# ibm-granite/dolomite-engine

Measured on NVIDIA H100. Metric: tokens_per_sec, higher is better.
Workload: dtype bf16

## Files before the change

dolomite_engine_b200/_lib.py:

```python

from __future__ import annotations

import ctypes
import os
from ctypes import c_char_p, c_float, c_int, c_int64, c_uint32, c_void_p

_HERE = os.path.dirname(os.path.abspath(__file__))
LIB_PATH = os.path.join(_HERE, "lib", "libdolomite_b200.so")


class DolomiteB200Error(RuntimeError):
    pass


_P = c_void_p
_I = c_int
_L = c_int64
_F = c_float
_U = c_uint32

SIGNATURES: dict[str, tuple] = {
    "dolomite_b200_last_error": (c_char_p, []),
    "dolomite_b200_abi_version": (_I, []),
    "dolomite_b200_device_info": (_I, [_P, _P, _P]),
    "dolomite_b200_set_option": (_I, [c_char_p, _I]),
    "dolomite_b200_get_option": (_I, [c_char_p, _P]),
    "dolomite_b200_rmsnorm_fwd": (_I, [_P, _P, _P, _P, _L, _I, _F, _P]),
    "dolomite_b200_rmsnorm_bwd_workspace_bytes": (_L, [_I]),
    "dolomite_b200_rmsnorm_bwd": (_I, [_P, _P, _P, _P, _P, _P, _P, _P, _L, _I, _P]),
    "dolomite_b200_rope_qk_inplace": (_I, [_P, _L, _L, _I, _I, _I, _P, _P, _P, _I, _L, _I, _P]),
    "dolomite_b200_layernorm_fwd": (_I, [_P, _P, _P, _P, _P, _P, _L, _I, _F, _P]),
    "dolomite_b200_layernorm_bwd_workspace_bytes": (_L, [_I]),
    "dolomite_b200_layernorm_bwd": (_I, [_P, _P, _P, _P, _P, _P, _P, _P, _P, _P, _L, _I, _P]),
    "dolomite_b200_act_fwd": (_I, [_I, _I, _P, _P, _L, _L, _P]),
    "dolomite_b200_act_bwd": (_I, [_I, _I, _P, _P, _P, _P, _L, _L, _P]),
    "dolomite_b200_act_bwd_segmented": (_I, [_I, _I, _P, _P, _P, _P, _L, _L, _P, _I, _P]),
    "dolomite_b200_gelu_fwd": (_I, [_P, _P, _L, _P]),
    "dolomite_b200_gelu_bwd": (_I, [_P, _P, _P, _P, _L, _L, _P]),
    "dolomite_b200_swiglu_fwd": (_I, [_P, _P, _L, _L, _P]),
    "dolomite_b200_swiglu_bwd": (_I, [_P, _P, _P, _L, _L, _P]),
    "dolomite_b200_swiglu_bwd_bias": (_I, [_P, _P, _P, _P, _L, _L, _P]),
    "dolomite_b200_embedding_fwd": (_I, [_P, _P, _P, _L, _I, _L, _F, _P]),
    "dolomite_b200_embedding_bwd": (_I, [_P, _P, _P, _L, _I, _L, _F, _P]),
    "dolomite_b200_cross_entropy_fwd_bwd": (_I, [_P, _L, _P, _P, _P, _P, _P, _L, _L, _L, _F, _F, _P]),
    "dolomite_b200_cross_entropy_count": (_I, [_P, _L, _L, _P, _P]),
    "dolomite_b200_cross_entropy_rows": (_I, [_P, _L, _P, _P, _P, _P, _L, _L, _L, _F, _F, _P]),
    "dolomite_b200_cross_entropy_mean": (_I, [_P, _L, _P, _P, _P]),
    "dolomite_b200_colsum_accum": (_I, [_P, _L, _P, _L, _L, _F, _P]),
    "dolomite_b200_colsum_accum_segmented": (_I, [_P, _L, _P, _L, _L, _P, _I, _F, _P]),
    "dolomite_b200_scale_bf16_by_device_scalar": (_I, [_P, _L, _P, _P]),
    "dolomite_b200_add_scaled": (_I, [_P, _P, _P, _F, _L, _P]),
    "dolomite_b200_dropout_fwd": (_I, [_P, _P, _P, _L, _F, _F, _U, _U, _P]),
    "dolomite_b200_dropout_bwd": (_I, [_P, _P, _L, _F, _F, _U, _U, _P]),
    "dolomite_b200_sumsq_workspace_bytes": (_L, []),
    "dolomite_b200_sumsq_accum": (_I, [_P, _L, _P, _P, _P]),
    "dolomite_b200_clip_coef": (_I, [_P, _F, _P, _P, _P]),
    "dolomite_b200_adamw_step": (_I, [_P, _P, _P, _P, _P, _L, _F, _F, _F, _F, _F, _L, _P, _P]),
    "dolomite_b200_cast_f32_to_bf16": (_I, [_P, _P, _L, _P]),
    "dolomite_b200_accum_bf16_into_f32": (_I, [_P, _P, _F, _L, _P]),
    "dolomite_b200_gemm_bf16": (
        _I,
        [_P, _L, _I, _P, _L, _I, _P, _L, _I, _P, _L, _F, _F, _P, _L, _L, _L, _I, _P],
    ),
    "dolomite_b200_gemm_bf16_wgrad_multi": (_I, [_I, _P, _P, _P, _P, _P, _P, _P, _P, _L, _P, _P, _P]),
    "dolomite_b200_gemm_bf16_tile_n": (_I, [_I, _P, _P, _P, _P]),
    "dolomite_b200_gemm_fp8": (
        _I,
        [_P, _L, _I, _P, _L, _I, _P, _P, _P, _L, _I, _P, _L, _F, _F, _P, _L, _L, _L, _I, _P],
    ),
    "dolomite_b200_gemm_fp8_wgrad_multi": (
        _I,
        [_I, _P, _P, _P, _P, _P, _P, _P, _P, _P, _P, _L, _P, _P, _I, _I, _I, _P],
    ),
    "dolomite_b200_fp8_cast": (_I, [_P, _L, _L, _L, _I, _P, _P, _P, _P, _P]),
    "dolomite_b200_fp8_scaling_update": (_I, [_P, _I, _L, _P, _P, _F, _P]),
    "dolomite_b200_gemm_bf16_grouped_m": (_I, [_P, _L, _P, _L, _I, _P, _L, _F, _L, _L, _L, _P, _I, _I, _P]),
    "dolomite_b200_gemm_bf16_grouped_k": (_I, [_P, _L, _P, _L, _P, _L, _F, _F, _L, _L, _L, _P, _I, _P]),
    "dolomite_b200_moe_max_rows": (_L, [_L, _I, _I]),
    "dolomite_b200_moe_route": (_I, [_P, _L, _I, _I, _P, _P, _P, _P, _P, _P, _P, _P, _P, _P]),
    "dolomite_b200_gemm_bf16_grouped_m_gather": (_I, [_P, _L, _L, _P, _P, _L, _P, _L, _F, _L, _L, _L, _P, _I, _I, _P]),
    "dolomite_b200_gemm_bf16_grouped_m_bias": (
        _I,
        [_P, _L, _L, _P, _P, _L, _I, _P, _L, _P, _L, _F, _L, _L, _L, _P, _I, _I, _P],
    ),
    "dolomite_b200_moe_gather": (_I, [_P, _P, _P, _P, _L, _I, _I, _I, _P]),
    "dolomite_b200_moe_combine": (_I, [_P, _P, _P, _P, _P, _L, _I, _I, _F, _P]),
    "dolomite_b200_moe_combine_bwd": (_I, [_P, _P, _P, _P, _P, _P, _P, _L, _I, _I, _I, _F, _P]),
    "dolomite_b200_moe_token_sum": (_I, [_P, _P, _P, _L, _I, _I, _P]),
    "dolomite_b200_moe_router_bwd": (_I, [_P, _P, _P, _P, _L, _I, _I, _P]),
    "dolomite_b200_moe_aux_partial_floats": (_L, [_L, _I]),
    "dolomite_b200_moe_aux_stats": (_I, [_P, _P, _L, _L, _I, _I, _P, _P, _P]),
    "dolomite_b200_moe_aux_finalize": (_I, [_P, _I, _L, _F, _P, _P, _P, _P]),
    "dolomite_b200_moe_router_bwd_aux": (_I, [_P, _P, _P, _P, _P, _P, _P, _L, _L, _I, _I, _P]),
    "dolomite_b200_attn_varlen_fwd": (_I, [_P, _L, _P, _P, _P, _I, _L, _I, _I, _I, _I, _F, _P]),
    "dolomite_b200_attn_decode": (_I, [_P, _L, _P, _P, _P, _P, _I, _L, _I, _I, _I, _F, _P]),
    "dolomite_b200_attn_varlen_bwd_workspace_bytes": (_L, [_L, _I, _I, _I]),
    "dolomite_b200_attn_varlen_bwd": (
        _I,
        [_P, _P, _L, _P, _P, _P, _P, _I, _L, _I, _I, _I, _I, _F, _P, _P],
    ),
    "dolomite_b200_attn_varlen_fwd_dropout": (_I, [_P, _L, _P, _P, _P, _I, _L, _I, _I, _I, _I, _F, _F, _U, _U, _P]),
    "dolomite_b200_attn_varlen_bwd_dropout": (
        _I,
        [_P, _P, _L, _P, _P, _P, _P, _I, _L, _I, _I, _I, _I, _F, _F, _U, _U, _P, _P],
    ),
    "dolomite_b200_attn_varlen_fwd_alibi": (_I, [_P, _L, _P, _P, _P, _I, _L, _I, _I, _I, _I, _F, _F, _U, _U, _P, _P]),
    "dolomite_b200_attn_varlen_bwd_alibi": (
        _I,
        [_P, _P, _L, _P, _P, _P, _P, _I, _L, _I, _I, _I, _I, _F, _F, _U, _U, _P, _P, _P],
    ),
    "dolomite_b200_attn_decode_alibi": (_I, [_P, _L, _P, _P, _P, _P, _I, _L, _I, _I, _I, _F, _P, _P]),
}

_lib = None


def lib_available() -> bool:
    return os.path.exists(LIB_PATH)


def load():
    global _lib
    if _lib is not None:
        return _lib
    if not os.path.exists(LIB_PATH):
        raise DolomiteB200Error(
            f"{LIB_PATH} not found. Build it with `python -m dolomite_engine_b200.build` "
            "(or __graft_entry__.build()); there is no CPU / PyTorch fallback for the hot path."
        )
    lib = ctypes.CDLL(LIB_PATH)
    for name, (res, args) in SIGNATURES.items():
        fn = getattr(lib, name)
        fn.restype = res
        fn.argtypes = args
    _lib = lib
    for item in filter(None, os.environ.get("DOLO_OPTIONS", "").split(",")):
        key, _, value = item.partition("=")
        if lib.dolomite_b200_set_option(key.strip().encode(), int(value)) != 0:
            raise DolomiteB200Error(f"DOLO_OPTIONS: {lib.dolomite_b200_last_error().decode()}")
    return lib


def check(rc: int, what: str = "") -> None:
    if rc != 0:
        msg = load().dolomite_b200_last_error()
        raise DolomiteB200Error(f"{what}: rc={rc}: {msg.decode() if msg else '?'}")


KERNELS_PER_CALL = {
    "dolomite_b200_rmsnorm_fwd": 1, "dolomite_b200_rmsnorm_bwd": 2, "dolomite_b200_rope_qk_inplace": 1,
    "dolomite_b200_layernorm_fwd": 1, "dolomite_b200_layernorm_bwd": 3, "dolomite_b200_gelu_fwd": 1,
    "dolomite_b200_gelu_bwd": 1, "dolomite_b200_swiglu_fwd": 1, "dolomite_b200_swiglu_bwd": 1, "dolomite_b200_swiglu_bwd_bias": 1,
    "dolomite_b200_act_fwd": 1, "dolomite_b200_act_bwd": 1,
    "dolomite_b200_embedding_fwd": 1,
    "dolomite_b200_embedding_bwd": 1, "dolomite_b200_cross_entropy_fwd_bwd": 3, "dolomite_b200_colsum_accum": 1,
    "dolomite_b200_scale_bf16_by_device_scalar": 1, "dolomite_b200_add_scaled": 1, "dolomite_b200_sumsq_accum": 2,
    "dolomite_b200_clip_coef": 1, "dolomite_b200_adamw_step": 1, "dolomite_b200_cast_f32_to_bf16": 1,
    "dolomite_b200_accum_bf16_into_f32": 1, "dolomite_b200_gemm_bf16": 1, "dolomite_b200_attn_varlen_fwd": 1,
    "dolomite_b200_attn_varlen_bwd": 3, "dolomite_b200_attn_varlen_fwd_dropout": 1, "dolomite_b200_attn_varlen_bwd_dropout": 3,
    "dolomite_b200_attn_varlen_fwd_alibi": 1, "dolomite_b200_attn_varlen_bwd_alibi": 3, "dolomite_b200_attn_decode_alibi": 1,
    "dolomite_b200_dropout_fwd": 1, "dolomite_b200_dropout_bwd": 1, "dolomite_b200_gemm_bf16_tile_n": 0,
    "dolomite_b200_moe_aux_stats": 2,
}
launch_counts: dict[str, int] = {}


def reset_launch_counts() -> None:
    launch_counts.clear()


def total_kernel_launches() -> int:
    return sum(KERNELS_PER_CALL.get(k, 1) * v for k, v in launch_counts.items())


def call(name: str, *args):
    lib = load()
    launch_counts[name] = launch_counts.get(name, 0) + 1
    rc = getattr(lib, name)(*args)
    if rc != 0:
        msg = lib.dolomite_b200_last_error()
        raise DolomiteB200Error(f"{name} failed (rc={rc}): {msg.decode() if msg else '?'}")
```

dolomite_engine_b200/csrc/gemm.cu:

```cuda
#include <string.h>

#include "common.cuh"
#include "wgmma.cuh"
#include "../../include/dolomite_b200.h"

using namespace dolo;

namespace {

constexpr int BM = 128;
constexpr int BN = 128;
constexpr int BK = 64;
constexpr int A_STAGE_BYTES = BM * BK * 2;
constexpr int GEMM_THREADS = 384;

constexpr int EPI_SLAB_BYTES = 64 * 128;
constexpr int EPI_BYTES = 2  * 2  * EPI_SLAB_BYTES;
constexpr int EPI_BIAS_BYTES = 2  * 256 * 2;

template <int TN>
struct Ring {
    static_assert(TN == 128 || TN == 256, "tile width 128 or 256");
    static constexpr int STAGES = TN == 256 ? 4 : 6;
    static constexpr int B_BYTES = TN * BK * 2;
    static constexpr int STAGE_BYTES = A_STAGE_BYTES + B_BYTES;
    static constexpr int EPI_OFFSET = STAGES * STAGE_BYTES;
    static constexpr int BIAS_OFFSET = EPI_OFFSET + EPI_BYTES;
    static constexpr int BAR_OFFSET = BIAS_OFFSET + EPI_BIAS_BYTES;
    static constexpr int SMEM_BYTES = 1024  + BAR_OFFSET + 256 ;
    static_assert(EPI_OFFSET % 1024 == 0, "epilogue slabs must stay 1024-byte aligned");
    static_assert((2 * STAGES + 4) * 8 <= 256, "barrier area");
    static_assert(SMEM_BYTES <= 232448, "shared memory budget exceeded (227 KB per block on sm_90)");
};

constexpr int PRODUCER_REGS = 40;
constexpr int CONSUMER_REGS = 232;
static_assert(PRODUCER_REGS * 128 + 2 * CONSUMER_REGS * 128 <= 65536, "register file exceeded");

constexpr double TILE256_COST = 1.65;

constexpr int MAXP = 4;

struct GemmMaps {
    CUtensorMap a[MAXP], b[MAXP], d[MAXP], c[MAXP];
};

struct Problem {
    void* D;
    const void* C;
    const __nv_bfloat16* bias;
    int64_t ldd, ldc;
    int M, N;
    int num_m, num_n, num_kb;
    int group_m;
    int tile_start;
    float alpha, beta;
    uint64_t hint_a, hint_b;
};

struct GemmParams {
    Problem pr[MAXP];
    int n_prob;
    int num_tiles;
    int d_is_f32;
    int grouped;
    const int* m_tile_group;
    const int* a_row_index;
    const void* gather_a;
    int64_t gather_lda;
    int gather_k;
    int b_group_rows;
    const int* group_k_offsets;
    int num_groups;
    int64_t bias_group_stride;
    const float* a_scale_inv[MAXP];
    const float* b_scale_inv[MAXP];
};

struct TileInfo {
    int q;
    int m_blk, n_blk, grp, kb0, kb1;
    bool valid;
};

__device__ __forceinline__ void tile_coords(int t, int num_m, int num_n, int gm, int& m_blk, int& n_blk) {
    const int per_group = gm * num_n;
    const int group = t / per_group;
    const int first_m = group * gm;
    const int gsize = min(num_m - first_m, gm);
    const int r = t - group * per_group;
    m_blk = first_m + r % gsize;
    n_blk = r / gsize;
}

template <bool GROUPED>
__device__ __forceinline__ TileInfo tile_info(int t, const GemmParams& p) {
    TileInfo ti;
    ti.q = 0;
#pragma unroll
    for (int i = 1; i < MAXP; ++i)
        if (i < p.n_prob && t >= p.pr[i].tile_start) ti.q = i;
    const Problem& pr = p.pr[ti.q];
    t -= pr.tile_start;
    ti.grp = 0;
    ti.kb0 = 0;
    ti.kb1 = pr.num_kb;
    ti.valid = true;
    if (GROUPED && p.grouped == 3) {
        const int per = pr.num_m * pr.num_n;
        const int split = t / per;
        tile_coords(t - split * per, pr.num_m, pr.num_n, pr.group_m, ti.m_blk, ti.n_blk);
        const int kb_per = (pr.num_kb + p.num_groups - 1) / p.num_groups;
        ti.kb0 = split * kb_per;
        ti.kb1 = min(pr.num_kb, ti.kb0 + kb_per);
        ti.valid = ti.kb1 > ti.kb0;
    } else if (GROUPED && p.grouped == 2) {
        const int per = pr.num_m * pr.num_n;
        ti.grp = t / per;
        tile_coords(t - ti.grp * per, pr.num_m, pr.num_n, pr.group_m, ti.m_blk, ti.n_blk);
        ti.kb0 = p.group_k_offsets[ti.grp] / BK;
        ti.kb1 = p.group_k_offsets[ti.grp + 1] / BK;
        ti.valid = ti.kb1 > ti.kb0;
    } else {
        tile_coords(t, pr.num_m, pr.num_n, pr.group_m, ti.m_blk, ti.n_blk);
        if (GROUPED && p.grouped == 1) {
            ti.grp = p.m_tile_group[ti.m_blk];
            ti.valid = ti.grp >= 0;
        }
    }
    return ti;
}

struct Epilogue {
    uint8_t* slabs;
    uint32_t* bias;
    uint64_t* c_bar;
    int slab = 0;
    uint32_t c_phase = 0;
    int cw;
    bool leader;

    __device__ __forceinline__ void load_c_prefetch(const CUtensorMap* cmap, int chunk_cols, int col0, int row0, int grp) {
        tma_store_wait_read<0>();
#pragma unroll
        for (int i = 0; i < 2; ++i) {
            const int s = slab ^ i;
            mbar_expect_tx(&c_bar[s], EPI_SLAB_BYTES);
            tma_load_3d(slabs + s * EPI_SLAB_BYTES, cmap, &c_bar[s], col0 + i * chunk_cols, row0, grp);
        }
    }

    __device__ __forceinline__ void begin_tile() {
        if (leader) tma_store_wait_read<0>();
        named_bar_sync(1 + cw, 128);
    }

    __device__ __forceinline__ void reuse_slab(bool has_c, const CUtensorMap* cmap, int col, int row0, int grp) {
        if (leader) {
            tma_store_wait_read<1>();
            if (has_c) {
                mbar_expect_tx(&c_bar[slab], EPI_SLAB_BYTES);
                tma_load_3d(slabs + slab * EPI_SLAB_BYTES, cmap, &c_bar[slab], col, row0, grp);
            }
        }
        named_bar_sync(1 + cw, 128);
    }

    template <int TN, bool F32, bool SCALED>
    __device__ __forceinline__ void store(const float (&acc)[TN / 2], const CUtensorMap* dmap, const CUtensorMap* cmap,
                                          int col0, int row0, int grp, float s, float alpha, float beta, bool has_bias,
                                          bool has_c, bool reduce) {
        constexpr int CHUNK = F32 ? 32 : 64;
        constexpr int NB = CHUNK / 8;
        const int lane = threadIdx.x & 31;
        const int wrow = ((threadIdx.x >> 5) & 3) * 16;
        auto scaled = [s](float a) { return SCALED ? s * a : a; };
#pragma unroll
        for (int ch = 0; ch < TN / CHUNK; ++ch) {
            uint8_t* sl = slabs + slab * EPI_SLAB_BYTES;
            if (ch >= 2) reuse_slab(has_c, cmap, col0 + ch * CHUNK, row0, grp);
            if (has_c) {
                mbar_wait(&c_bar[slab], (c_phase >> slab) & 1u, 4);
                c_phase ^= 1u << slab;
            }
            if constexpr (F32) {
#pragma unroll
                for (int jj = 0; jj < NB; ++jj) {
                    const int j = ch * NB + jj;
                    float b0 = 0.f, b1 = 0.f;
                    if (has_bias) {
                        const uint32_t bv = bias[4 * j + (lane & 3)];
                        b0 = bf16_lo(bv);
                        b1 = bf16_hi(bv);
                    }
#pragma unroll
                    for (int h = 0; h < 2; ++h) {
                        const int r = wrow + 8 * h + (lane >> 2);
                        const int byte = jj * 32 + (lane & 3) * 8;
                        float2* d = reinterpret_cast<float2*>(sl + r * 128 + ((((byte >> 4) ^ (r & 7)) << 4) | (byte & 15)));
                        float v0 = (scaled(acc[4 * j + 2 * h]) + b0) * alpha;
                        float v1 = (scaled(acc[4 * j + 2 * h + 1]) + b1) * alpha;
                        if (has_c) {
                            const float2 c2 = *d;
                            v0 += beta * c2.x;
                            v1 += beta * c2.y;
                        }
                        *d = make_float2(v0, v1);
                    }
                }
            } else {
                const int m = lane >> 3;
                const int r = wrow + 8 * (m & 1) + (lane & 7);
#pragma unroll
                for (int jj = 0; jj < NB; jj += 2) {
                    const uint32_t addr = smem_u32(sl + r * 128 + (((jj + (m >> 1)) ^ (lane & 7)) << 4));
                    uint32_t cv[4], out[4];
                    if (has_c) ldmatrix_x4(addr, cv);
#pragma unroll
                    for (int i = 0; i < 4; ++i) {
                        const int j = ch * NB + jj + (i >> 1), h = i & 1;
                        float b0 = 0.f, b1 = 0.f;
                        if (has_bias) {
                            const uint32_t bv = bias[4 * j + (lane & 3)];
                            b0 = bf16_lo(bv);
                            b1 = bf16_hi(bv);
                        }
                        float v0 = (scaled(acc[4 * j + 2 * h]) + b0) * alpha;
                        float v1 = (scaled(acc[4 * j + 2 * h + 1]) + b1) * alpha;
                        if (has_c) {
                            v0 += beta * bf16_lo(cv[i]);
                            v1 += beta * bf16_hi(cv[i]);
                        }
                        out[i] = pack_bf16(v0, v1);
                    }
                    stmatrix_x4(addr, out);
                }
            }
            issue(dmap, col0 + ch * CHUNK, row0, grp, reduce);
        }
    }

    template <int TN>
    __device__ __forceinline__ void store_zero_f32(const CUtensorMap* dmap, int col0, int row0, int grp) {
        begin_tile();
#pragma unroll 1
        for (int ch = 0; ch < TN / 32; ++ch) {
            if (ch >= 2) reuse_slab(false, nullptr, 0, 0, 0);
            uint4* s = reinterpret_cast<uint4*>(slabs + slab * EPI_SLAB_BYTES);
#pragma unroll
            for (int i = 0; i < EPI_SLAB_BYTES / 16 / 128; ++i) s[(threadIdx.x & 127) + 128 * i] = make_uint4(0u, 0u, 0u, 0u);
            issue(dmap, col0 + ch * 32, row0, grp, false);
        }
    }

    __device__ __forceinline__ void issue(const CUtensorMap* dmap, int col, int row0, int grp, bool reduce) {
        const uint8_t* sl = slabs + slab * EPI_SLAB_BYTES;
        fence_proxy_async_smem();
        named_bar_sync(1 + cw, 128);
        if (leader) {
            if (reduce)
                tma_reduce_add_3d(dmap, sl, col, row0, grp);
            else
                tma_store_3d(dmap, sl, col, row0, grp);
            tma_store_commit();
        }
        slab ^= 1;
    }
};

template <bool A_MN_, bool B_MN_>
struct Bf16Ops {
    static constexpr bool A_MN = A_MN_, B_MN = B_MN_;
    static constexpr int KB_ELEMS = BK;
    static constexpr bool SPLIT = false, SCALED = false, GROUPED = true;
    template <int TN>
    static __device__ __forceinline__ void mma(float (&acc)[TN / 2], uint64_t adesc, uint64_t bdesc, uint32_t scale_d) {
        wgmma_ss<TN, A_MN ? 1 : 0, B_MN ? 1 : 0>(acc, adesc, bdesc, scale_d);
    }
};

template <int FA, int FB, bool SPLIT_>
struct Fp8Ops {
    static constexpr bool A_MN = false, B_MN = false;
    static constexpr int KB_ELEMS = 128;
    static constexpr bool SPLIT = SPLIT_, SCALED = true, GROUPED = false;
    template <int TN>
    static __device__ __forceinline__ void mma(float (&acc)[TN / 2], uint64_t adesc, uint64_t bdesc, uint32_t scale_d) {
        static_assert(TN == 128, "fp8 tiles are 128 wide");
        wgmma_fp8_n128<FA, FB>(acc, adesc, bdesc, scale_d);
    }
};

template <class Op, int TN>
__device__ __forceinline__ void gemm_body(const GemmMaps& maps, const GemmParams& p) {
    constexpr bool A_MN = Op::A_MN, B_MN = Op::B_MN;
    constexpr int STAGES = Ring<TN>::STAGES;
    constexpr int B_STAGE_BYTES = Ring<TN>::B_BYTES;
    constexpr int STAGE_BYTES = Ring<TN>::STAGE_BYTES;
    extern __shared__ uint8_t smem_raw[];
    uint8_t* smem = smem_align_1024(smem_raw);
    uint8_t* smem_a = smem;
    uint8_t* smem_b = smem + STAGES * A_STAGE_BYTES;
    uint64_t* bars = reinterpret_cast<uint64_t*>(smem + Ring<TN>::BAR_OFFSET);
    uint64_t* full_bar = bars;
    uint64_t* empty_bar = bars + STAGES;
    uint64_t* c_bar = bars + 2 * STAGES;

    const int wg = threadIdx.x >> 7;
    const int warp = threadIdx.x >> 5;
    const int lane = threadIdx.x & 31;
    const int num_tiles = p.num_tiles;
    const bool gather = Op::GROUPED && TN == 128 && !A_MN && p.a_row_index != nullptr;

    if (threadIdx.x == 0) {
        for (int q = 0; q < p.n_prob; ++q) {
            if (!gather) tma_prefetch_desc(&maps.a[q]);
            tma_prefetch_desc(&maps.b[q]);
        }
        for (int i = 0; i < STAGES; ++i) {
            mbar_init(&full_bar[i], gather ? 33 : 1);
            mbar_init(&empty_bar[i], 8);
        }
        for (int i = 0; i < 4; ++i) mbar_init(&c_bar[i], 1);
        mbar_fence_init();
    }
    __syncthreads();

    if (wg == 0) {
        if constexpr (TN == 256) setmaxnreg_dec<PRODUCER_REGS>();
        if (warp != 0) return;
        if (gather) {
            const __nv_bfloat16* A = static_cast<const __nv_bfloat16*>(p.gather_a);
            int stage = 0;
            uint32_t phase = 0;
            for (int t = blockIdx.x; t < num_tiles; t += gridDim.x) {
                const TileInfo ti = tile_info<Op::GROUPED>(t, p);
                if (!ti.valid) continue;
                const CUtensorMap* tmap_b = &maps.b[ti.q];
                const int b_outer = ti.grp * p.b_group_rows;
                const int4 src = *reinterpret_cast<const int4*>(p.a_row_index + int64_t(ti.m_blk) * BM + lane * 4);
                const int srow[4] = {src.x, src.y, src.z, src.w};
                for (int kb = ti.kb0; kb < ti.kb1; ++kb) {
                    mbar_wait(&empty_bar[stage], phase ^ 1, 1);
                    uint8_t* sa = smem_a + stage * A_STAGE_BYTES;
                    uint8_t* sb = smem_b + stage * B_STAGE_BYTES;
                    if (lane == 0) {
                        mbar_expect_tx(&full_bar[stage], B_STAGE_BYTES);
                        if (!B_MN) {
                            tma_load_2d(sb, tmap_b, &full_bar[stage], kb * BK, b_outer + ti.n_blk * BN);
                        } else {
#pragma unroll
                            for (int i = 0; i < BN / 64; ++i)
                                tma_load_2d(sb + i * (BK * 128), tmap_b, &full_bar[stage], ti.n_blk * BN + i * 64,
                                            b_outer + kb * BK);
                        }
                    }
#pragma unroll
                    for (int i = 0; i < 4; ++i) {
                        const int r = lane * 4 + i;
                        const __nv_bfloat16* g = A + int64_t(srow[i]) * p.gather_lda + int64_t(kb) * BK;
#pragma unroll
                        for (int c = 0; c < 8; ++c) {
                            uint4 v = make_uint4(0u, 0u, 0u, 0u);
                            if (kb * BK + c * 8 < p.gather_k) v = __ldg(reinterpret_cast<const uint4*>(g + c * 8));
                            *reinterpret_cast<uint4*>(sa + r * 128 + ((c ^ (r & 7)) << 4)) = v;
                        }
                    }
                    fence_proxy_async_smem();
                    mbar_arrive(&full_bar[stage]);
                    if (++stage == STAGES) { stage = 0; phase ^= 1; }
                }
            }
        } else if (elect_one()) {
            int stage = 0;
            uint32_t phase = 0;
            for (int t = blockIdx.x; t < num_tiles; t += gridDim.x) {
                const TileInfo ti = tile_info<Op::GROUPED>(t, p);
                if (!ti.valid) continue;
                const CUtensorMap* tmap_a = &maps.a[ti.q];
                const CUtensorMap* tmap_b = &maps.b[ti.q];
                const uint64_t ha = p.pr[ti.q].hint_a, hb = p.pr[ti.q].hint_b;
                const int m_blk = ti.m_blk, n_blk = ti.n_blk;
                const int b_outer = (Op::GROUPED && p.grouped == 1) ? ti.grp * p.b_group_rows : 0;
                for (int kb = ti.kb0; kb < ti.kb1; ++kb) {
                    mbar_wait(&empty_bar[stage], phase ^ 1, 1);
                    uint8_t* sa = smem_a + stage * A_STAGE_BYTES;
                    uint8_t* sb = smem_b + stage * B_STAGE_BYTES;
                    mbar_expect_tx(&full_bar[stage], STAGE_BYTES);
                    if (!A_MN) {
                        tma_load_2d_hint(sa, tmap_a, &full_bar[stage], kb * Op::KB_ELEMS, m_blk * BM, ha);
                    } else {
#pragma unroll
                        for (int i = 0; i < BM / 64; ++i)
                            tma_load_2d_hint(sa + i * (BK * 128), tmap_a, &full_bar[stage], m_blk * BM + i * 64, kb * BK, ha);
                    }
                    if (!B_MN) {
                        tma_load_2d_hint(sb, tmap_b, &full_bar[stage], kb * Op::KB_ELEMS, b_outer + n_blk * TN, hb);
                    } else {
#pragma unroll
                        for (int i = 0; i < TN / 64; ++i)
                            tma_load_2d_hint(sb + i * (BK * 128), tmap_b, &full_bar[stage], n_blk * TN + i * 64,
                                             b_outer + kb * BK, hb);
                    }
                    if (++stage == STAGES) { stage = 0; phase ^= 1; }
                }
            }
        }
        return;
    }

    if constexpr (TN == 256) setmaxnreg_inc<CONSUMER_REGS>();
    const int cw = wg - 1;
    const int wt = threadIdx.x & 127;
    Epilogue epi;
    epi.slabs = smem + Ring<TN>::EPI_OFFSET + cw * 2 * EPI_SLAB_BYTES;
    epi.bias = reinterpret_cast<uint32_t*>(smem + Ring<TN>::BIAS_OFFSET + cw * (EPI_BIAS_BYTES / 2));
    epi.c_bar = c_bar + 2 * cw;
    epi.cw = cw;
    epi.leader = wt == 0;
    const int chunk_cols = p.d_is_f32 ? 32 : 64;
    int stage = 0;
    uint32_t phase = 0;
    float acc[TN / 2];
    float tot[TN / 2];
    for (int t = blockIdx.x; t < num_tiles; t += gridDim.x) {
        const TileInfo ti = tile_info<Op::GROUPED>(t, p);
        const Problem& pr = p.pr[ti.q];
        const int row0 = ti.m_blk * BM + cw * 64;
        const int col0 = ti.n_blk * TN;
        const int dgrp = Op::GROUPED && p.grouped == 2 ? ti.grp : 0;
        if (!ti.valid) {
            if (Op::GROUPED && p.grouped == 2 && p.d_is_f32 && pr.C == nullptr) epi.store_zero_f32<TN>(&maps.d[ti.q], col0, row0, dgrp);
            continue;
        }
        const bool has_bias = pr.bias != nullptr;
        const bool has_c = pr.C != nullptr;
        uint32_t bias_v = 0;
        if (has_bias && wt < TN / 2 && col0 + 2 * wt < pr.N) {
            const __nv_bfloat16* brow = pr.bias + ti.grp * p.bias_group_stride;
            if (col0 + 2 * wt + 1 < pr.N)
                bias_v = __ldg(reinterpret_cast<const uint32_t*>(brow + col0 + 2 * wt));
            else
                bias_v = __bfloat16_as_ushort(brow[col0 + 2 * wt]);
        }
        int prev_stage = -1;
        for (int kb = ti.kb0; kb < ti.kb1; ++kb) {
            mbar_wait(&full_bar[stage], phase, 3);
            wgmma_fence();
            const uint32_t sa = smem_u32(smem_a + stage * A_STAGE_BYTES);
            const uint32_t sb = smem_u32(smem_b + stage * B_STAGE_BYTES);
#pragma unroll
            for (int k = 0; k < 4; ++k) {
                const uint64_t adesc = A_MN ? gmma_desc(sa + cw * (BK * 128) + k * 2048, BK * 128, 1024, 1)
                                            : gmma_desc(sa + cw * (64 * 128) + k * 32, 16, 1024, 1);
                const uint64_t bdesc = B_MN ? gmma_desc(sb + k * 2048, BK * 128, 1024, 1)
                                            : gmma_desc(sb + k * 32, 16, 1024, 1);
                Op::template mma<TN>(acc, adesc, bdesc, ((!Op::SPLIT && kb != ti.kb0) || k != 0) ? 1u : 0u);
            }
            wgmma_commit();
            if (kb == min(ti.kb0 + 2, ti.kb1 - 1) && has_c && epi.leader) epi.load_c_prefetch(&maps.c[ti.q], chunk_cols, col0, row0, dgrp);
            if constexpr (Op::SPLIT) {
                wgmma_wait<0>();
                reg_fence<TN / 2>(acc);
                if (lane == 0) mbar_arrive(&empty_bar[stage]);
                if (kb == ti.kb0) {
#pragma unroll
                    for (int i = 0; i < TN / 2; ++i) tot[i] = acc[i];
                } else {
#pragma unroll
                    for (int i = 0; i < TN / 2; ++i) tot[i] += acc[i];
                }
            } else {
                wgmma_wait<1>();
                if (prev_stage >= 0 && lane == 0) mbar_arrive(&empty_bar[prev_stage]);
                prev_stage = stage;
            }
            if (++stage == STAGES) { stage = 0; phase ^= 1; }
        }
        if constexpr (!Op::SPLIT) {
            wgmma_wait<0>();
            reg_fence<TN / 2>(acc);
            if (prev_stage >= 0 && lane == 0) mbar_arrive(&empty_bar[prev_stage]);
        }
        const float(&res)[TN / 2] = Op::SPLIT ? tot : acc;
        float s = 1.f;
        if constexpr (Op::SCALED) s = __ldg(p.a_scale_inv[ti.q]) * __ldg(p.b_scale_inv[ti.q]);
        if (has_bias && wt < TN / 2) epi.bias[wt] = bias_v;
        epi.begin_tile();

        if (p.d_is_f32)
            epi.store<TN, true, Op::SCALED>(res, &maps.d[ti.q], &maps.c[ti.q], col0, row0, dgrp, s, pr.alpha, pr.beta,
                                            has_bias, has_c, Op::GROUPED && p.grouped == 3);
        else
            epi.store<TN, false, Op::SCALED>(res, &maps.d[ti.q], &maps.c[ti.q], col0, row0, dgrp, s, pr.alpha, pr.beta,
                                             has_bias, has_c, false);
    }
    if (epi.leader) tma_store_wait_all<0>();
}

template <bool A_MN, bool B_MN, int TN>
__global__ void __launch_bounds__(GEMM_THREADS, 1)
    gemm_bf16_kernel(const __grid_constant__ GemmMaps maps, const __grid_constant__ GemmParams p) {
    gemm_body<Bf16Ops<A_MN, B_MN>, TN>(maps, p);
}

template <int FA, int FB, bool SPLIT>
__global__ void __launch_bounds__(GEMM_THREADS, 1)
    gemm_fp8_kernel(const __grid_constant__ GemmMaps maps, const __grid_constant__ GemmParams p) {
    gemm_body<Fp8Ops<FA, FB, SPLIT>, 128>(maps, p);
}

int gemm_workers() {
    const int sms = dolo_num_sms() - dolo_option_gemm_sm_margin();
    return sms < 1 ? 1 : sms;
}

template <int TN, void (*KERNEL)(GemmMaps, GemmParams)>
int launch_gemm(const GemmMaps& maps, const GemmParams& p, cudaStream_t st) {
    constexpr int smem_bytes = Ring<TN>::SMEM_BYTES;
    static bool attr_set = false;
    if (!attr_set) {
        DOLO_CUDA_OK(cudaFuncSetAttribute(KERNEL, cudaFuncAttributeMaxDynamicSharedMemorySize, smem_bytes));
        attr_set = true;
    }
    const int sms = gemm_workers();
    const int grid = p.num_tiles < sms ? p.num_tiles : sms;
    KERNEL<<<grid, GEMM_THREADS, smem_bytes, st>>>(maps, p);
    DOLO_LAUNCH_OK("gemm");
    return DOLO_OK;
}

int choose_tile_n(int n, const int64_t* M, const int64_t* N) {
    const int forced = dolo_option_gemm_tile_n();
    if (forced != 0) return forced;
    const int64_t w = gemm_workers();
    int64_t t128 = 0, t256 = 0;
    for (int q = 0; q < n; ++q) {
        const int64_t mb = (M[q] + BM - 1) / BM;
        t128 += mb * ((N[q] + 127) / 128);
        t256 += mb * ((N[q] + 255) / 256);
    }
    const double c128 = double((t128 + w - 1) / w);
    const double c256 = double((t256 + w - 1) / w) * TILE256_COST;
    return c256 < c128 ? 256 : 128;
}

}

struct GroupArgs {
    int mode = 0;
    const int* a_row_index = nullptr;
    int64_t a_rows = 0;
    const int* m_tile_group = nullptr;
    int64_t b_group_rows = 0;
    const int* group_k_offsets = nullptr;
    int num_groups = 1;
    int64_t d_group_stride = 0;
    int64_t b_total_outer = 0;
    int64_t bias_group_stride = 0;
};

struct GemmProblemArgs {
    const void* A; int64_t lda;
    const void* B; int64_t ldb;
    void* D; int64_t ldd;
    const void* C; int64_t ldc;
    const void* bias;
    float alpha, beta;
    int64_t M, N, K;
    const float* a_scale_inv = nullptr;
    const float* b_scale_inv = nullptr;
};

static int setup_problem(GemmMaps& maps, GemmParams& p, int q, const GemmProblemArgs& g, int ab, int a_mn_major,
                         int b_mn_major, int d_is_f32, const GroupArgs& ga, int tile_n) {
    const int64_t M = g.M, N = g.N, K = g.K;
    if (ab == 1) {
        DOLO_REQUIRE(M > 0 && N > 0 && K > 0, "gemm_fp8: empty problem (M=%lld N=%lld K=%lld)", (long long)M,
                     (long long)N, (long long)K);
        DOLO_REQUIRE(K % 16 == 0 && N % 16 == 0, "gemm_fp8: K=%lld and N=%lld must be multiples of 16", (long long)K,
                     (long long)N);
        DOLO_REQUIRE(g.lda % 16 == 0 && g.ldb % 16 == 0 && g.lda >= K && g.ldb >= K,
                     "gemm_fp8: lda / ldb must be >= K and multiples of 16 (16-byte aligned fp8 rows)");
        DOLO_REQUIRE(g.a_scale_inv != nullptr && g.b_scale_inv != nullptr, "gemm_fp8: missing scale_inv pointer");
        p.a_scale_inv[q] = g.a_scale_inv;
        p.b_scale_inv[q] = g.b_scale_inv;
    }
    DOLO_REQUIRE(K > 0, "gemm: K must be > 0");
    DOLO_REQUIRE(g.lda * ab % 16 == 0 && g.ldb * ab % 16 == 0 && g.ldd % (d_is_f32 ? 4 : 8) == 0,
                 "gemm: leading dimensions must keep 16-byte alignment");
    {
        const int64_t per = d_is_f32 ? 4 : 8;
        DOLO_REQUIRE(g.ldd >= (N + per - 1) / per * per,
                     "gemm: ldd=%lld must cover N=%lld rounded up to 16 bytes (the TMA store writes that segment)",
                     (long long)g.ldd, (long long)N);
    }
    DOLO_REQUIRE(g.C == nullptr || g.ldc % (d_is_f32 ? 4 : 8) == 0, "gemm: ldc alignment");
    DOLO_REQUIRE((reinterpret_cast<uintptr_t>(g.bias) & 3) == 0, "gemm: bias must be 4-byte aligned");
    DOLO_REQUIRE(M < (1ll << 31) && N < (1ll << 31) && K < (1ll << 31), "gemm: dimension too large");
    uint64_t dims[2], strides[2];
    uint32_t box[2];
    int rc;
    if (ga.a_row_index != nullptr) {
        DOLO_REQUIRE(!a_mn_major, "gemm: gather-on-load needs a K-major A");
        DOLO_REQUIRE((reinterpret_cast<uintptr_t>(g.A) & 15) == 0, "gemm: gather-on-load needs a 16-byte aligned A");
        DOLO_REQUIRE(K % 8 == 0, "gemm: gather-on-load needs K %% 8 == 0 (K=%lld)", (long long)K);
        p.gather_a = g.A;
        p.gather_lda = g.lda;
        p.gather_k = int(K);
    } else {
        if (!a_mn_major) {
            dims[0] = uint64_t(K); dims[1] = uint64_t(M); strides[0] = ab; strides[1] = uint64_t(g.lda) * ab;
            box[0] = 128 / ab; box[1] = BM;
        } else {
            dims[0] = uint64_t(M); dims[1] = uint64_t(K); strides[0] = 2; strides[1] = uint64_t(g.lda) * 2;
            box[0] = 64; box[1] = BK;
        }
        rc = dolo_make_tmap(&maps.a[q], g.A, ab, 2, dims, strides, box, DOLO_SW_128);
        if (rc) return rc;
    }
    strides[0] = ab;
    if (!b_mn_major) {
        dims[0] = uint64_t(K); dims[1] = uint64_t(ga.mode == 1 ? ga.b_total_outer : N); strides[1] = uint64_t(g.ldb) * ab;
        box[0] = 128 / ab; box[1] = uint32_t(tile_n);
    } else {
        dims[0] = uint64_t(N); dims[1] = uint64_t(ga.mode == 1 ? ga.b_total_outer : K); strides[1] = uint64_t(g.ldb) * 2;
        box[0] = 64; box[1] = BK;
    }
    rc = dolo_make_tmap(&maps.b[q], g.B, ab, 2, dims, strides, box, DOLO_SW_128);
    if (rc) return rc;
    {
        const uint64_t eb = d_is_f32 ? 4 : 2;
        const int64_t groups = ga.mode == 2 ? ga.num_groups : 1;
        const int64_t group_stride = ga.mode == 2 ? ga.d_group_stride : M * g.ldd;
        uint64_t ddims[3] = {uint64_t(N), uint64_t(M), uint64_t(groups)};
        uint64_t dstrides[3] = {eb, uint64_t(g.ldd) * eb, uint64_t(group_stride) * eb};
        const uint32_t dbox[3] = {uint32_t(128 / eb), 64, 1};
        rc = dolo_make_tmap(&maps.d[q], g.D, int(eb), 3, ddims, dstrides, dbox, DOLO_SW_128);
        if (rc) return rc;
        if (g.C != nullptr) {
            dstrides[1] = uint64_t(g.ldc) * eb;
            if (ga.mode != 2) dstrides[2] = uint64_t(M * g.ldc) * eb;
            rc = dolo_make_tmap(&maps.c[q], g.C, int(eb), 3, ddims, dstrides, dbox, DOLO_SW_128);
            if (rc) return rc;
        }
    }
    Problem& pr = p.pr[q];
    pr.D = g.D;
    pr.C = g.C;
    pr.bias = static_cast<const __nv_bfloat16*>(g.bias);
    pr.ldd = g.ldd;
    pr.ldc = g.ldc;
    pr.M = int(M);
    pr.N = int(N);
    pr.alpha = g.alpha;
    pr.beta = g.C ? g.beta : 0.f;
    pr.hint_a = pr.hint_b = TMA_HINT_NORMAL;
    if (ab == 2 && dolo_option_gemm_l2_hints() && ga.mode == 0 && K >= 4096 && (M + N) * K * 2 > (24ll << 20)) {
        const bool a_smaller = M <= N;
        pr.hint_a = a_smaller ? TMA_HINT_EVICT_LAST : TMA_HINT_EVICT_FIRST;
        pr.hint_b = a_smaller ? TMA_HINT_EVICT_FIRST : TMA_HINT_EVICT_LAST;
    }
    pr.num_m = int((M + BM - 1) / BM);
    pr.num_n = int((N + tile_n - 1) / tile_n);
    pr.num_kb = int((K * ab + 127) / 128);
    {
        const int64_t panel_bytes = int64_t(BM) * K * ab;
        int64_t gm = (12ll << 20) / (panel_bytes > 0 ? panel_bytes : 1);
        if (gm < 4) gm = 4;
        if (gm > 64) gm = 64;
        pr.group_m = int(gm);
    }
    return DOLO_OK;
}

template <int TN>
static int dispatch_layout(int a_mn_major, int b_mn_major, const GemmMaps& maps, const GemmParams& p, cudaStream_t st) {
    if (!a_mn_major && !b_mn_major) return launch_gemm<TN, gemm_bf16_kernel<false, false, TN>>(maps, p, st);
    if (!a_mn_major && b_mn_major) return launch_gemm<TN, gemm_bf16_kernel<false, true, TN>>(maps, p, st);
    if (a_mn_major && !b_mn_major) return launch_gemm<TN, gemm_bf16_kernel<true, false, TN>>(maps, p, st);
    return launch_gemm<TN, gemm_bf16_kernel<true, true, TN>>(maps, p, st);
}

static int dispatch(int tile_n, int a_mn_major, int b_mn_major, const GemmMaps& maps, const GemmParams& p, cudaStream_t st) {
    return tile_n == 256 ? dispatch_layout<256>(a_mn_major, b_mn_major, maps, p, st)
                         : dispatch_layout<128>(a_mn_major, b_mn_major, maps, p, st);
}

template <int FA, int FB>
static int dispatch_fp8_split(int split, const GemmMaps& maps, const GemmParams& p, cudaStream_t st) {
    return split ? launch_gemm<BN, gemm_fp8_kernel<FA, FB, true>>(maps, p, st)
                 : launch_gemm<BN, gemm_fp8_kernel<FA, FB, false>>(maps, p, st);
}

static int dispatch_fp8(int a_fmt, int b_fmt, int split, const GemmMaps& maps, const GemmParams& p, cudaStream_t st) {
    if (a_fmt == 0 && b_fmt == 0) return dispatch_fp8_split<0, 0>(split, maps, p, st);
    if (a_fmt == 0 && b_fmt == 1) return dispatch_fp8_split<0, 1>(split, maps, p, st);
    if (a_fmt == 1 && b_fmt == 0) return dispatch_fp8_split<1, 0>(split, maps, p, st);
    return dispatch_fp8_split<1, 1>(split, maps, p, st);
}

static int gemm_impl(const void* A, int64_t lda, int a_mn_major, const void* B, int64_t ldb, int b_mn_major, void* D,
                     int64_t ldd, int d_is_f32, const void* C, int64_t ldc, float alpha, float beta, const void* bias,
                     int64_t M, int64_t N, int64_t K, int flags, void* stream, const GroupArgs& ga) {
    DOLO_REQUIRE(M >= 0 && N >= 0 && K >= 0, "gemm: negative dimension");
    if (M == 0 || N == 0) return DOLO_OK;
    const bool tma_store = (flags & DOLO_GEMM_FLAG_TMA_STORE) != 0;
    DOLO_REQUIRE(!tma_store || (!d_is_f32 && C == nullptr), "gemm: TMA-store epilogue needs bf16 D and no C");
    const int tile_n = ga.mode == 0 ? choose_tile_n(1, &M, &N) : BN;
    GemmMaps maps;
    GemmParams p;
    memset(&p, 0, sizeof(p));
    GemmProblemArgs g{A, lda, B, ldb, D, ldd, C, ldc, bias, alpha, beta, M, N, K};
    int rc = setup_problem(maps, p, 0, g, 2, a_mn_major, b_mn_major, d_is_f32, ga, tile_n);
    if (rc) return rc;
    p.n_prob = 1;
    p.pr[0].tile_start = 0;
    p.num_tiles = p.pr[0].num_m * p.pr[0].num_n * (ga.mode >= 2 ? ga.num_groups : 1);
    p.d_is_f32 = d_is_f32;
    p.grouped = ga.mode;
    p.m_tile_group = ga.m_tile_group;
    p.a_row_index = ga.a_row_index;
    p.b_group_rows = int(ga.b_group_rows);
    p.group_k_offsets = ga.group_k_offsets;
    p.num_groups = ga.num_groups;
    p.bias_group_stride = ga.bias_group_stride;
    return dispatch(tile_n, a_mn_major, b_mn_major, maps, p, static_cast<cudaStream_t>(stream));
}

extern "C" int dolomite_b200_gemm_bf16_wgrad_multi(int n_problems, const void* const* dY, const int64_t* ld_dy,
                                                   const void* const* X, const int64_t* ld_x, float* const* dW,
                                                   const int64_t* ld_dw, const int64_t* M, const int64_t* N, int64_t K,
                                                   const float* alpha, const int* accumulate, void* stream) {
    DOLO_REQUIRE(n_problems >= 1 && n_problems <= MAXP, "wgrad_multi: between 1 and %d problems per launch", MAXP);
    for (int q = 0; q < n_problems; ++q) DOLO_REQUIRE(M[q] > 0 && N[q] > 0, "wgrad_multi: empty problem %d", q);
    const int tile_n = choose_tile_n(n_problems, M, N);
    GemmMaps maps;
    GemmParams p;
    memset(&p, 0, sizeof(p));
    int tiles = 0;
    for (int q = 0; q < n_problems; ++q) {
        GemmProblemArgs g{dY[q], ld_dy[q], X[q], ld_x[q], dW[q], ld_dw[q], accumulate[q] ? dW[q] : nullptr, ld_dw[q], nullptr,
                          alpha[q], 1.f, M[q], N[q], K};
        int rc = setup_problem(maps, p, q, g, 2, 1, 1, 1, GroupArgs(), tile_n);
        if (rc) return rc;
        p.pr[q].tile_start = tiles;
        tiles += p.pr[q].num_m * p.pr[q].num_n;
    }
    p.n_prob = n_problems;
    p.num_tiles = tiles;
    p.d_is_f32 = 1;
    p.grouped = 0;
    p.num_groups = 1;
    return dispatch(tile_n, 1, 1, maps, p, static_cast<cudaStream_t>(stream));
}

extern "C" int dolomite_b200_gemm_bf16_tile_n(int n_problems, const int64_t* M, const int64_t* N, int* tile_n,
                                              float* cost_256_over_128) {
    DOLO_REQUIRE(n_problems >= 1 && n_problems <= MAXP && M != nullptr && N != nullptr && tile_n != nullptr,
                 "gemm_bf16_tile_n: between 1 and %d problems, non-null M, N and tile_n", MAXP);
    *tile_n = choose_tile_n(n_problems, M, N);
    if (cost_256_over_128 != nullptr) *cost_256_over_128 = float(TILE256_COST);
    return DOLO_OK;
}

extern "C" int dolomite_b200_gemm_bf16(const void* A, int64_t lda, int a_mn_major, const void* B, int64_t ldb,
                                       int b_mn_major, void* D, int64_t ldd, int d_is_f32, const void* C, int64_t ldc,
                                       float alpha, float beta, const void* bias, int64_t M, int64_t N, int64_t K,
                                       int flags, void* stream) {
    if (flags & DOLO_GEMM_FLAG_SPLITK_ACCUMULATE) {
        DOLO_REQUIRE(d_is_f32 && bias == nullptr && (C == nullptr || (C == D && beta == 1.f)),
                     "gemm: split-K accumulate needs fp32 D, no bias and C == D with beta == 1");
        const int64_t tiles = ((M + BM - 1) / BM) * ((N + BN - 1) / BN);
        const int64_t num_kb = (K + BK - 1) / BK;
        const int sms = dolo_num_sms();
        int best_s = 1;
        double best = 1e30;
        for (int s = 1; s <= 16; ++s) {
            if (s > 1 && num_kb / s < 8) break;
            const double waves = double((tiles * s + sms - 1) / sms) / double(s);
            if (waves < best - 1e-9) { best = waves; best_s = s; }
        }
        GroupArgs ga;
        ga.mode = 3;
        ga.num_groups = best_s;
        return gemm_impl(A, lda, a_mn_major, B, ldb, b_mn_major, D, ldd, 1, nullptr, 0, alpha, 0.f, nullptr, M, N, K, 0,
                         stream, ga);
    }
    return gemm_impl(A, lda, a_mn_major, B, ldb, b_mn_major, D, ldd, d_is_f32, C, ldc, alpha, beta, bias, M, N, K, flags,
                     stream, GroupArgs());
}

static int grouped_m_impl(const void* A, int64_t lda, int64_t a_rows, const int32_t* a_row_index, const void* B,
                          int64_t ldb, int b_mn_major, void* D, int64_t ldd, const void* bias, int64_t ld_bias,
                          float alpha, int64_t M_max, int64_t N, int64_t K, const int32_t* m_tile_group, int num_groups,
                          int flags, void* stream) {
    DOLO_REQUIRE(M_max % BM == 0, "grouped gemm: M_max=%lld must be a multiple of %d (padded expert segments)",
                 (long long)M_max, BM);
    DOLO_REQUIRE(!b_mn_major || K % BK == 0, "grouped gemm: MN-major B needs K %% %d == 0", BK);
    DOLO_REQUIRE(m_tile_group != nullptr && num_groups > 0, "grouped gemm: missing group table");
    if (a_row_index != nullptr) {
        DOLO_REQUIRE(!b_mn_major && a_rows > 0, "grouped gemm (gather): K-major B and a_rows > 0 needed");
        DOLO_REQUIRE((reinterpret_cast<uintptr_t>(a_row_index) & 15) == 0,
                     "grouped gemm (gather): row index must be 16-byte aligned");
    }
    DOLO_REQUIRE(bias == nullptr || (ld_bias >= N && ld_bias % 2 == 0),
                 "grouped gemm: ld_bias=%lld must be even and >= N=%lld", (long long)ld_bias, (long long)N);
    GroupArgs ga;
    ga.mode = 1;
    ga.a_row_index = a_row_index;
    ga.a_rows = a_rows;
    ga.m_tile_group = m_tile_group;
    ga.num_groups = num_groups;
    ga.b_group_rows = b_mn_major ? K : N;
    ga.b_total_outer = ga.b_group_rows * num_groups;
    ga.bias_group_stride = bias != nullptr ? ld_bias : 0;
    return gemm_impl(A, lda, 0, B, ldb, b_mn_major, D, ldd, 0, nullptr, 0, alpha, 0.f, bias, M_max, N, K, flags, stream,
                     ga);
}

extern "C" int dolomite_b200_gemm_bf16_grouped_m(const void* A, int64_t lda, const void* B, int64_t ldb, int b_mn_major,
                                                 void* D, int64_t ldd, float alpha, int64_t M_max, int64_t N, int64_t K,
                                                 const int32_t* m_tile_group, int num_groups, int flags, void* stream) {
    return grouped_m_impl(A, lda, 0, nullptr, B, ldb, b_mn_major, D, ldd, nullptr, 0, alpha, M_max, N, K, m_tile_group,
                          num_groups, flags, stream);
}

extern "C" int dolomite_b200_gemm_bf16_grouped_m_gather(const void* A, int64_t lda, int64_t a_rows,
                                                        const int32_t* a_row_index, const void* B, int64_t ldb, void* D,
                                                        int64_t ldd, float alpha, int64_t M_max, int64_t N, int64_t K,
                                                        const int32_t* m_tile_group, int num_groups, int flags,
                                                        void* stream) {
    DOLO_REQUIRE(a_row_index != nullptr, "grouped gemm (gather): missing row index");
    return grouped_m_impl(A, lda, a_rows, a_row_index, B, ldb, 0, D, ldd, nullptr, 0, alpha, M_max, N, K, m_tile_group,
                          num_groups, flags, stream);
}

extern "C" int dolomite_b200_gemm_bf16_grouped_m_bias(const void* A, int64_t lda, int64_t a_rows,
                                                      const int32_t* a_row_index, const void* B, int64_t ldb,
                                                      int b_mn_major, void* D, int64_t ldd, const void* bias,
                                                      int64_t ld_bias, float alpha, int64_t M_max, int64_t N, int64_t K,
                                                      const int32_t* m_tile_group, int num_groups, int flags,
                                                      void* stream) {
    DOLO_REQUIRE(bias != nullptr, "grouped gemm (bias): missing bias");
    return grouped_m_impl(A, lda, a_rows, a_row_index, B, ldb, b_mn_major, D, ldd, bias, ld_bias, alpha, M_max, N, K,
                          m_tile_group, num_groups, flags, stream);
}

extern "C" int dolomite_b200_gemm_bf16_grouped_k(const void* A, int64_t lda, const void* B, int64_t ldb, float* D,
                                                 int64_t ldd, float alpha, float beta, int64_t M, int64_t N,
                                                 int64_t K_max, const int32_t* group_k_offsets, int num_groups,
                                                 void* stream) {
    DOLO_REQUIRE(group_k_offsets != nullptr && num_groups > 0, "grouped wgrad: missing offsets");
    GroupArgs ga;
    ga.mode = 2;
    ga.group_k_offsets = group_k_offsets;
    ga.num_groups = num_groups;
    ga.d_group_stride = M * ldd;
    return gemm_impl(A, lda, 1, B, ldb, 1, D, ldd, 1, beta != 0.f ? D : nullptr, ldd, alpha, beta, nullptr, M, N, K_max, 0,
                     stream, ga);
}

extern "C" int dolomite_b200_gemm_fp8(const void* A, int64_t lda, int a_fmt, const void* B, int64_t ldb, int b_fmt,
                                      const float* a_scale_inv, const float* b_scale_inv, void* D, int64_t ldd,
                                      int d_is_f32, const void* C, int64_t ldc, float alpha, float beta, const void* bias,
                                      int64_t M, int64_t N, int64_t K, int split_accumulate, void* stream) {
    DOLO_REQUIRE(M >= 0 && N >= 0 && K >= 0, "gemm_fp8: negative dimension");
    DOLO_REQUIRE((a_fmt == 0 || a_fmt == 1) && (b_fmt == 0 || b_fmt == 1), "gemm_fp8: format must be 0 (e4m3) or 1 (e5m2)");
    if (M == 0 || N == 0) return DOLO_OK;
    GemmMaps maps;
    GemmParams p;
    memset(&p, 0, sizeof(p));
    GemmProblemArgs g{A, lda, B, ldb, D, ldd, C, ldc, bias, alpha, beta, M, N, K, a_scale_inv, b_scale_inv};
    int rc = setup_problem(maps, p, 0, g, 1, 0, 0, d_is_f32, GroupArgs(), BN);
    if (rc) return rc;
    p.n_prob = 1;
    p.num_tiles = p.pr[0].num_m * p.pr[0].num_n;
    p.d_is_f32 = d_is_f32;
    p.num_groups = 1;
    return dispatch_fp8(a_fmt, b_fmt, split_accumulate, maps, p, static_cast<cudaStream_t>(stream));
}

extern "C" int dolomite_b200_gemm_fp8_wgrad_multi(int n_problems, const void* const* dYt, const int64_t* ld_dyt,
                                                  const void* const* Xt, const int64_t* ld_xt,
                                                  const float* const* dy_scale_inv, const float* const* x_scale_inv,
                                                  float* const* dW, const int64_t* ld_dw, const int64_t* M,
                                                  const int64_t* N, int64_t K, const float* alpha, const int* accumulate,
                                                  int dy_fmt, int x_fmt, int split_accumulate, void* stream) {
    DOLO_REQUIRE(n_problems >= 1 && n_problems <= MAXP, "gemm_fp8_wgrad_multi: between 1 and %d problems per launch", MAXP);
    DOLO_REQUIRE((dy_fmt == 0 || dy_fmt == 1) && (x_fmt == 0 || x_fmt == 1),
                 "gemm_fp8_wgrad_multi: format must be 0 (e4m3) or 1 (e5m2)");
    GemmMaps maps;
    GemmParams p;
    memset(&p, 0, sizeof(p));
    int tiles = 0;
    for (int q = 0; q < n_problems; ++q) {
        GemmProblemArgs g{dYt[q], ld_dyt[q], Xt[q], ld_xt[q], dW[q], ld_dw[q], accumulate[q] ? dW[q] : nullptr, ld_dw[q],
                          nullptr, alpha[q], 1.f, M[q], N[q], K, dy_scale_inv[q], x_scale_inv[q]};
        int rc = setup_problem(maps, p, q, g, 1, 0, 0, 1, GroupArgs(), BN);
        if (rc) return rc;
        p.pr[q].tile_start = tiles;
        tiles += p.pr[q].num_m * p.pr[q].num_n;
    }
    p.n_prob = n_problems;
    p.num_tiles = tiles;
    p.d_is_f32 = 1;
    p.num_groups = 1;
    return dispatch_fp8(dy_fmt, x_fmt, split_accumulate, maps, p, static_cast<cudaStream_t>(stream));
}
```

dolomite_engine_b200/kernels.py:

```python

from __future__ import annotations

import torch

from . import _lib

_BF16 = torch.bfloat16


def set_option(key: str, value: int) -> None:
    _lib.call("dolomite_b200_set_option", key.encode(), int(value))


def get_option(key: str) -> int:
    import ctypes

    v = ctypes.c_int(0)
    _lib.call("dolomite_b200_get_option", key.encode(), ctypes.addressof(v))
    return int(v.value)


def _stream() -> int:
    return torch.cuda.current_stream().cuda_stream


def _ptr(t: torch.Tensor | None) -> int | None:
    return None if t is None else t.data_ptr()


def _req(t: torch.Tensor, dtype, name: str) -> None:
    if not t.is_cuda:
        raise _lib.DolomiteB200Error(f"{name} must be a CUDA tensor (no CPU fallback on the hot path)")
    if t.dtype != dtype:
        raise _lib.DolomiteB200Error(f"{name} must be {dtype}, got {t.dtype}")


def rows_empty(rows: int, cols: int, dtype=_BF16, device=None) -> torch.Tensor:
    per = 16 // torch.empty((), dtype=dtype).element_size()
    ld = -(-cols // per) * per
    if ld == cols:
        return torch.empty(rows, cols, dtype=dtype, device=device)
    return torch.empty(rows, ld, dtype=dtype, device=device)[:, :cols]


def rows_aligned(t: torch.Tensor) -> torch.Tensor:
    per = 16 // t.element_size()
    if t.stride(1) == 1 and t.stride(0) % per == 0 and t.data_ptr() % 16 == 0:
        return t
    out = rows_empty(t.shape[0], t.shape[1], t.dtype, t.device)
    out.copy_(t)
    return out


def rmsnorm_fwd(x: torch.Tensor, w: torch.Tensor, eps: float, out: torch.Tensor | None = None):
    _req(x, _BF16, "x"), _req(w, _BF16, "w")
    assert x.is_contiguous() and x.dim() == 2
    T, H = x.shape
    y = torch.empty_like(x) if out is None else out
    rstd = torch.empty(T, dtype=torch.float32, device=x.device)
    _lib.call("dolomite_b200_rmsnorm_fwd", x.data_ptr(), w.data_ptr(), y.data_ptr(), rstd.data_ptr(), T, H, eps, _stream())
    return y, rstd


_ws_cache: dict = {}


def _workspace(nbytes: int, device) -> torch.Tensor:
    key = (device, "ws")
    buf = _ws_cache.get(key)
    if buf is None or buf.numel() < nbytes:
        buf = torch.empty(max(nbytes, 1 << 20), dtype=torch.uint8, device=device)
        _ws_cache[key] = buf
    return buf


def rmsnorm_bwd(dy, x, w, rstd, dw_accum: torch.Tensor | None, dx_add: torch.Tensor | None = None, out=None):
    _req(dy, _BF16, "dy"), _req(x, _BF16, "x")
    T, H = x.shape
    dx = torch.empty_like(x) if out is None else out
    ws = _workspace(_lib.load().dolomite_b200_rmsnorm_bwd_workspace_bytes(H), x.device)
    if dw_accum is not None:
        _req(dw_accum, torch.float32, "dw_accum")
    _lib.call(
        "dolomite_b200_rmsnorm_bwd", dy.data_ptr(), x.data_ptr(), w.data_ptr(), rstd.data_ptr(), _ptr(dx_add),
        dx.data_ptr(), _ptr(dw_accum), ws.data_ptr(), T, H, _stream(),
    )
    return dx


def rope_qk_inplace(qkv, n_groups: int, q_per_group: int, head_dim: int, cos, sin, position_ids, inverse=False):
    _req(qkv, _BF16, "qkv"), _req(cos, _BF16, "cos"), _req(sin, _BF16, "sin")
    assert qkv.dim() == 2 and qkv.stride(1) == 1
    assert position_ids.dtype in (torch.int32, torch.int64) and position_ids.is_contiguous()
    T = qkv.shape[0]
    _lib.call(
        "dolomite_b200_rope_qk_inplace", qkv.data_ptr(), qkv.stride(0), T, n_groups, q_per_group, head_dim,
        cos.data_ptr(), sin.data_ptr(), position_ids.data_ptr(), int(position_ids.dtype == torch.int64),
        cos.shape[0], int(inverse), _stream(),
    )
    return qkv


def layernorm_fwd(x, w, b, eps: float, out=None):
    _req(x, _BF16, "x"), _req(w, _BF16, "w")
    T, H = x.shape
    y = torch.empty_like(x) if out is None else out
    mean = torch.empty(T, dtype=torch.float32, device=x.device)
    rstd = torch.empty(T, dtype=torch.float32, device=x.device)
    _lib.call("dolomite_b200_layernorm_fwd", x.data_ptr(), w.data_ptr(), _ptr(b), y.data_ptr(), mean.data_ptr(), rstd.data_ptr(),
              T, H, eps, _stream())
    return y, mean, rstd


def layernorm_bwd(dy, x, w, mean, rstd, dw_accum, db_accum, dx_add=None, out=None):
    _req(dy, _BF16, "dy"), _req(x, _BF16, "x")
    T, H = x.shape
    dx = torch.empty_like(x) if out is None else out
    ws = _workspace(_lib.load().dolomite_b200_layernorm_bwd_workspace_bytes(H), x.device)
    _lib.call("dolomite_b200_layernorm_bwd", dy.data_ptr(), x.data_ptr(), w.data_ptr(), mean.data_ptr(), rstd.data_ptr(),
              _ptr(dx_add), dx.data_ptr(), _ptr(dw_accum), _ptr(db_accum), ws.data_ptr(), T, H, _stream())
    return dx


def act_fwd(x, act_id: int, form: int, out=None):
    _req(x, _BF16, "x")
    T, W = x.shape
    F = W if form == 0 else W // 2
    y = torch.empty(T, F, dtype=_BF16, device=x.device) if out is None else out
    _lib.call("dolomite_b200_act_fwd", act_id, form, x.data_ptr(), y.data_ptr(), T, F, _stream())
    return y


def act_bwd(dy, x, act_id: int, form: int, out=None, bias_grad_accum=None):
    _req(dy, _BF16, "dy"), _req(x, _BF16, "x")
    T, W = x.shape
    dx = torch.empty_like(x) if out is None else out
    if bias_grad_accum is not None:
        _req(bias_grad_accum, torch.float32, "bias_grad_accum")
        assert bias_grad_accum.numel() == W
    _lib.call("dolomite_b200_act_bwd", act_id, form, dy.data_ptr(), x.data_ptr(), dx.data_ptr(), _ptr(bias_grad_accum), T,
              W if form == 0 else W // 2, _stream())
    return dx


def act_bwd_segmented(dy, x, act_id: int, form: int, seg_offsets, bias_grad_accum, out=None):
    _req(dy, _BF16, "dy"), _req(x, _BF16, "x"), _req(bias_grad_accum, torch.float32, "bias_grad_accum")
    _req(seg_offsets, torch.int32, "seg_offsets")
    T, W = x.shape
    S = seg_offsets.numel() - 1
    assert bias_grad_accum.dim() == 2 and bias_grad_accum.shape == (S, W) and bias_grad_accum.stride(1) == 1
    dx = torch.empty_like(x) if out is None else out
    _lib.call("dolomite_b200_act_bwd_segmented", act_id, form, dy.data_ptr(), x.data_ptr(), dx.data_ptr(),
              bias_grad_accum.data_ptr(), bias_grad_accum.stride(0), W if form == 0 else W // 2, seg_offsets.data_ptr(), S,
              _stream())
    return dx


def gelu_fwd(x, out=None):
    _req(x, _BF16, "x")
    y = torch.empty_like(x) if out is None else out
    _lib.call("dolomite_b200_gelu_fwd", x.data_ptr(), y.data_ptr(), x.numel(), _stream())
    return y


def gelu_bwd(dy, x, out=None, bias_grad_accum=None):
    _req(dy, _BF16, "dy"), _req(x, _BF16, "x")
    T, F = x.shape
    dx = torch.empty_like(x) if out is None else out
    _lib.call("dolomite_b200_gelu_bwd", dy.data_ptr(), x.data_ptr(), dx.data_ptr(), _ptr(bias_grad_accum), T, F, _stream())
    return dx


def swiglu_fwd(x, out=None):
    _req(x, _BF16, "x")
    T, F2 = x.shape
    y = torch.empty(T, F2 // 2, dtype=_BF16, device=x.device) if out is None else out
    _lib.call("dolomite_b200_swiglu_fwd", x.data_ptr(), y.data_ptr(), T, F2 // 2, _stream())
    return y


def swiglu_bwd(dy, x, out=None, bias_grad_accum=None):
    _req(dy, _BF16, "dy"), _req(x, _BF16, "x")
    T, F2 = x.shape
    dx = torch.empty_like(x) if out is None else out
    if bias_grad_accum is not None:
        _req(bias_grad_accum, torch.float32, "bias_grad_accum")
        assert bias_grad_accum.numel() == F2
        _lib.call("dolomite_b200_swiglu_bwd_bias", dy.data_ptr(), x.data_ptr(), dx.data_ptr(), bias_grad_accum.data_ptr(),
                  T, F2 // 2, _stream())
    else:
        _lib.call("dolomite_b200_swiglu_bwd", dy.data_ptr(), x.data_ptr(), dx.data_ptr(), T, F2 // 2, _stream())
    return dx


def embedding_fwd(ids, wte, scale: float = 1.0, out=None):
    _req(ids, torch.int64, "ids"), _req(wte, _BF16, "wte")
    T = ids.numel()
    V, H = wte.shape
    y = torch.empty(T, H, dtype=_BF16, device=wte.device) if out is None else out
    _lib.call("dolomite_b200_embedding_fwd", ids.data_ptr(), wte.data_ptr(), y.data_ptr(), T, H, V, scale, _stream())
    return y


def embedding_bwd(ids, dout, dwte_accum, scale: float = 1.0):
    _req(ids, torch.int64, "ids"), _req(dout, _BF16, "dout"), _req(dwte_accum, torch.float32, "dwte")
    T = ids.numel()
    V, H = dwte_accum.shape
    _lib.call("dolomite_b200_embedding_bwd", ids.data_ptr(), dout.data_ptr(), dwte_accum.data_ptr(), T, H, V, scale, _stream())


def cross_entropy_fwd_bwd(logits, labels, ignore_index=-100, logit_scale=1.0, grad_scale=1.0, dlogits=None):
    _req(logits, _BF16, "logits"), _req(labels, torch.int64, "labels")
    T, V = logits.shape
    assert logits.stride(1) == 1
    dl = logits if dlogits is None else dlogits
    loss_tok = torch.empty(T, dtype=torch.float32, device=logits.device)
    loss = torch.empty(1, dtype=torch.float32, device=logits.device)
    scratch = torch.empty(2, dtype=torch.float32, device=logits.device)
    _lib.call(
        "dolomite_b200_cross_entropy_fwd_bwd", logits.data_ptr(), logits.stride(0), labels.data_ptr(), dl.data_ptr(),
        loss_tok.data_ptr(), loss.data_ptr(), scratch.data_ptr(), T, V, ignore_index, logit_scale, grad_scale, _stream(),
    )
    return loss, loss_tok, dl


def cross_entropy_count(labels, ignore_index=-100):
    _req(labels, torch.int64, "labels")
    scratch = torch.empty(2, dtype=torch.float32, device=labels.device)
    _lib.call("dolomite_b200_cross_entropy_count", labels.data_ptr(), labels.numel(), ignore_index, scratch.data_ptr(), _stream())
    return scratch


def cross_entropy_rows(logits, labels, loss_tok, scratch, ignore_index=-100, logit_scale=1.0, grad_scale=1.0):
    _req(logits, _BF16, "logits"), _req(labels, torch.int64, "labels"), _req(loss_tok, torch.float32, "loss_tok")
    t, V = logits.shape
    assert logits.stride(1) == 1 and labels.numel() == t and loss_tok.numel() == t
    _lib.call("dolomite_b200_cross_entropy_rows", logits.data_ptr(), logits.stride(0), labels.data_ptr(), logits.data_ptr(),
              loss_tok.data_ptr(), scratch.data_ptr(), t, V, ignore_index, logit_scale, grad_scale, _stream())
    return logits


def cross_entropy_mean(loss_tok, scratch):
    loss = torch.empty(1, dtype=torch.float32, device=loss_tok.device)
    _lib.call("dolomite_b200_cross_entropy_mean", loss_tok.data_ptr(), loss_tok.numel(), scratch.data_ptr(), loss.data_ptr(), _stream())
    return loss


def colsum_accum(x, out, scale: float = 1.0):
    _req(x, _BF16, "x"), _req(out, torch.float32, "out")
    T, N = x.shape
    _lib.call("dolomite_b200_colsum_accum", x.data_ptr(), x.stride(0), out.data_ptr(), T, N, scale, _stream())


def colsum_accum_segmented(x, seg_offsets, out, scale: float = 1.0):
    _req(x, _BF16, "x"), _req(out, torch.float32, "out"), _req(seg_offsets, torch.int32, "seg_offsets")
    T, N = x.shape
    S = seg_offsets.numel() - 1
    assert out.dim() == 2 and out.shape == (S, N) and out.stride(1) == 1 and x.stride(1) == 1
    _lib.call("dolomite_b200_colsum_accum_segmented", x.data_ptr(), x.stride(0), out.data_ptr(), out.stride(0), N,
              seg_offsets.data_ptr(), S, scale, _stream())


def scale_by_device_scalar(x, scale):
    _req(x, _BF16, "x"), _req(scale, torch.float32, "scale")
    n = x.numel()
    if not x.is_contiguous():
        assert x.dim() == 2 and x.stride(1) == 1 and x.stride(0) >= x.shape[1]
        n = x.shape[0] * x.stride(0)
        assert x.storage_offset() + n <= x.untyped_storage().nbytes() // x.element_size()
    _lib.call("dolomite_b200_scale_bf16_by_device_scalar", x.data_ptr(), n, scale.data_ptr(), _stream())


def add_scaled(a, b, alpha: float, out=None):
    _req(a, _BF16, "a"), _req(b, _BF16, "b")
    o = torch.empty_like(a) if out is None else out
    _lib.call("dolomite_b200_add_scaled", a.data_ptr(), b.data_ptr(), o.data_ptr(), alpha, a.numel(), _stream())
    return o


_M64 = (1 << 64) - 1


def dropout_keys(seed: int, site: int) -> tuple[int, int]:
    z = (int(seed) * 0x9E3779B97F4A7C15 + (int(site) + 1) * 0xD1B54A32D192ED03) & _M64
    z = ((z ^ (z >> 30)) * 0xBF58476D1CE4E5B9) & _M64
    z = ((z ^ (z >> 27)) * 0x94D049BB133111EB) & _M64
    z ^= z >> 31
    return int(z & 0xFFFFFFFF), int(z >> 32)


def dropout_fwd(x, p: float, keys: tuple[int, int], residual=None, post_mul: float = 1.0, out=None):
    _req(x, _BF16, "x")
    assert x.is_contiguous() and (residual is None or (residual.is_contiguous() and residual.shape == x.shape))
    o = torch.empty_like(x) if out is None else out
    _lib.call("dolomite_b200_dropout_fwd", x.data_ptr(), _ptr(residual), o.data_ptr(), x.numel(), float(p), float(post_mul),
              keys[0], keys[1], _stream())
    return o


def dropout_bwd(dy, p: float, keys: tuple[int, int], pre_mul: float = 1.0, out=None):
    _req(dy, _BF16, "dy")
    assert dy.is_contiguous()
    o = torch.empty_like(dy) if out is None else out
    _lib.call("dolomite_b200_dropout_bwd", dy.data_ptr(), o.data_ptr(), dy.numel(), float(p), float(pre_mul), keys[0], keys[1],
              _stream())
    return o


def sumsq_accum(g, out):
    _req(g, torch.float32, "g")
    ws = _workspace(_lib.load().dolomite_b200_sumsq_workspace_bytes(), g.device)
    _lib.call("dolomite_b200_sumsq_accum", g.data_ptr(), g.numel(), out.data_ptr(), ws.data_ptr(), _stream())


def clip_coef(sumsq, max_norm: float, coef_out, norm_out=None):
    _lib.call("dolomite_b200_clip_coef", sumsq.data_ptr(), float(max_norm), coef_out.data_ptr(), _ptr(norm_out), _stream())


def adamw_step(p, g, m, v, p_bf16, lr, beta1, beta2, eps, weight_decay, step, clip=None):
    _req(p, torch.float32, "p"), _req(g, torch.float32, "g")
    _lib.call(
        "dolomite_b200_adamw_step", p.data_ptr(), g.data_ptr(), m.data_ptr(), v.data_ptr(), _ptr(p_bf16), p.numel(),
        lr, beta1, beta2, eps, weight_decay, step, _ptr(clip), _stream(),
    )


def cast_f32_to_bf16(src, dst):
    _lib.call("dolomite_b200_cast_f32_to_bf16", src.data_ptr(), dst.data_ptr(), src.numel(), _stream())


def accum_bf16_into_f32(src, dst, scale=1.0):
    _lib.call("dolomite_b200_accum_bf16_into_f32", src.data_ptr(), dst.data_ptr(), scale, src.numel(), _stream())


GEMM_TMA_STORE = 1
GEMM_SPLITK_ACCUMULATE = 2
GEMM_DIRECT_EPILOGUE = 16
GEMM_F32_TMA_EPILOGUE = 32
wgrad_splitk = False
_default_gemm_flags = GEMM_TMA_STORE
gemm_timer = None


def set_default_gemm_flags(flags: int) -> None:
    global _default_gemm_flags
    _default_gemm_flags = flags


def gemm(a, b, *, a_mn=False, b_mn=False, out=None, out_dtype=_BF16, c=None, alpha=1.0, beta=0.0, bias=None, flags=None):
    _req(a, _BF16, "a"), _req(b, _BF16, "b")
    assert a.dim() == 2 and b.dim() == 2 and a.stride(1) == 1 and b.stride(1) == 1
    if a_mn:
        K, M = a.shape
    else:
        M, K = a.shape
    if b_mn:
        Kb, N = b.shape
    else:
        N, Kb = b.shape
    if K != Kb:
        raise _lib.DolomiteB200Error(f"gemm: contraction mismatch {K} vs {Kb}")
    if out is None:
        out = rows_empty(M, N, out_dtype, a.device)
    d_is_f32 = int(out.dtype == torch.float32)
    assert out.stride(1) == 1 and out.shape == (M, N)
    if c is not None:
        assert c.dtype == out.dtype and c.stride(1) == 1
    if flags is None:
        flags = _default_gemm_flags
        if d_is_f32 or c is not None:
            flags &= ~GEMM_TMA_STORE
        if d_is_f32 and c is out and beta == 1.0 and bias is None and wgrad_splitk:
            flags |= GEMM_SPLITK_ACCUMULATE
    if gemm_timer is not None:
        e0, e1 = torch.cuda.Event(enable_timing=True), torch.cuda.Event(enable_timing=True)
        e0.record()
    _lib.call(
        "dolomite_b200_gemm_bf16", a.data_ptr(), a.stride(0), int(a_mn), b.data_ptr(), b.stride(0), int(b_mn),
        out.data_ptr(), out.stride(0), d_is_f32, _ptr(c), 0 if c is None else c.stride(0), alpha, beta, _ptr(bias),
        M, N, K, flags, _stream(),
    )
    if gemm_timer is not None:
        e1.record()
        gemm_timer.append((2.0 * M * N * K, e0, e1))
    return out


def gemm_wgrad_multi(problems: list[tuple], n_rows: int | None = None) -> None:
    import ctypes

    n = len(problems)
    assert 1 <= n <= 4
    K = problems[0][0].shape[0] if n_rows is None else n_rows
    P, L, F, I = ctypes.c_void_p * n, ctypes.c_int64 * n, ctypes.c_float * n, ctypes.c_int * n
    for dy, x, dw, _, _ in problems:
        _req(dy, _BF16, "dy"), _req(x, _BF16, "x"), _req(dw, torch.float32, "dw")
        assert dy.shape[0] == K and x.shape[0] == K and dy.stride(1) == 1 and x.stride(1) == 1 and dw.stride(1) == 1
        assert dw.shape == (dy.shape[1], x.shape[1])
    if gemm_timer is not None:
        e0, e1 = torch.cuda.Event(enable_timing=True), torch.cuda.Event(enable_timing=True)
        e0.record()
    _lib.call(
        "dolomite_b200_gemm_bf16_wgrad_multi", n, P(*[q[0].data_ptr() for q in problems]), L(*[q[0].stride(0) for q in problems]),
        P(*[q[1].data_ptr() for q in problems]), L(*[q[1].stride(0) for q in problems]), P(*[q[2].data_ptr() for q in problems]),
        L(*[q[2].stride(0) for q in problems]), L(*[q[0].shape[1] for q in problems]), L(*[q[1].shape[1] for q in problems]),
        K, F(*[float(q[3]) for q in problems]), I(*[int(bool(q[4])) for q in problems]), _stream(),
    )
    if gemm_timer is not None:
        e1.record()
        gemm_timer.append((sum(2.0 * K * q[0].shape[1] * q[1].shape[1] for q in problems), e0, e1))


def gemm_tile_n(shapes: list[tuple[int, int]]) -> tuple[int, float]:
    import ctypes

    n = len(shapes)
    tile_n, cost = ctypes.c_int(0), ctypes.c_float(0.0)
    _lib.call("dolomite_b200_gemm_bf16_tile_n", n, (ctypes.c_int64 * n)(*[s[0] for s in shapes]),
              (ctypes.c_int64 * n)(*[s[1] for s in shapes]), ctypes.addressof(tile_n), ctypes.addressof(cost))
    return int(tile_n.value), float(cost.value)


E4M3, E5M2 = 0, 1
FP8_MAX = {E4M3: 448.0, E5M2: 57344.0}
_U8 = torch.uint8


def fp8_cast(x, fmt: int, scale, *, plain: bool = True, transpose: bool = False, amax=None, out=None, out_t=None):
    _req(x, _BF16, "x"), _req(scale, torch.float32, "scale")
    assert x.dim() == 2 and x.stride(1) == 1 and (plain or transpose)
    rows, cols = x.shape
    if plain and out is None:
        out = torch.empty(rows, cols, dtype=_U8, device=x.device)
    if transpose and out_t is None:
        out_t = torch.empty(cols, rows, dtype=_U8, device=x.device)
    if amax is not None:
        _req(amax, torch.float32, "amax")
    _lib.call("dolomite_b200_fp8_cast", x.data_ptr(), x.stride(0), rows, cols, fmt, scale.data_ptr(),
              _ptr(out) if plain else None, _ptr(out_t) if transpose else None, _ptr(amax), _stream())
    return (out if plain else None), (out_t if transpose else None)


def fp8_scaling_update(amax_history, scale, scale_inv, fmt: int) -> None:
    _req(amax_history, torch.float32, "amax_history"), _req(scale, torch.float32, "scale")
    _req(scale_inv, torch.float32, "scale_inv")
    L, n = amax_history.shape
    assert amax_history.is_contiguous() and scale.numel() == n and scale_inv.numel() == n
    _lib.call("dolomite_b200_fp8_scaling_update", amax_history.data_ptr(), L, n, scale.data_ptr(), scale_inv.data_ptr(),
              FP8_MAX[fmt], _stream())


def gemm_fp8(a, a_fmt: int, a_scale_inv, b, b_fmt: int, b_scale_inv, *, out=None, out_dtype=_BF16, c=None, alpha=1.0,
             beta=0.0, bias=None, split_accumulate: bool = False):
    _req(a, _U8, "a"), _req(b, _U8, "b"), _req(a_scale_inv, torch.float32, "a_scale_inv")
    _req(b_scale_inv, torch.float32, "b_scale_inv")
    assert a.dim() == 2 and b.dim() == 2 and a.stride(1) == 1 and b.stride(1) == 1
    M, K = a.shape
    N, Kb = b.shape
    if K != Kb:
        raise _lib.DolomiteB200Error(f"gemm_fp8: contraction mismatch {K} vs {Kb}")
    if out is None:
        out = torch.empty(M, N, dtype=out_dtype, device=a.device)
    assert out.stride(1) == 1 and out.shape == (M, N)
    if c is not None:
        assert c.dtype == out.dtype and c.stride(1) == 1
    if gemm_timer is not None:
        e0, e1 = torch.cuda.Event(enable_timing=True), torch.cuda.Event(enable_timing=True)
        e0.record()
    _lib.call(
        "dolomite_b200_gemm_fp8", a.data_ptr(), a.stride(0), a_fmt, b.data_ptr(), b.stride(0), b_fmt, a_scale_inv.data_ptr(),
        b_scale_inv.data_ptr(), out.data_ptr(), out.stride(0), int(out.dtype == torch.float32), _ptr(c),
        0 if c is None else c.stride(0), alpha, beta, _ptr(bias), M, N, K, int(split_accumulate), _stream(),
    )
    if gemm_timer is not None:
        e1.record()
        gemm_timer.append((2.0 * M * N * K, e0, e1))
    return out


def gemm_fp8_wgrad_multi(problems: list[tuple], dy_fmt: int = E5M2, x_fmt: int = E4M3, split_accumulate: bool = True):
    import ctypes

    n = len(problems)
    assert 1 <= n <= 4
    K = problems[0][0].shape[1]
    P, L, F, I = ctypes.c_void_p * n, ctypes.c_int64 * n, ctypes.c_float * n, ctypes.c_int * n
    for dyt, sdy, xt, sx, dw, _, _ in problems:
        _req(dyt, _U8, "dyt"), _req(xt, _U8, "xt"), _req(dw, torch.float32, "dw")
        assert dyt.shape[1] == K and xt.shape[1] == K and dyt.stride(1) == 1 and xt.stride(1) == 1 and dw.stride(1) == 1
        assert dw.shape == (dyt.shape[0], xt.shape[0])
    if gemm_timer is not None:
        e0, e1 = torch.cuda.Event(enable_timing=True), torch.cuda.Event(enable_timing=True)
        e0.record()
    _lib.call(
        "dolomite_b200_gemm_fp8_wgrad_multi", n, P(*[q[0].data_ptr() for q in problems]), L(*[q[0].stride(0) for q in problems]),
        P(*[q[2].data_ptr() for q in problems]), L(*[q[2].stride(0) for q in problems]),
        P(*[q[1].data_ptr() for q in problems]), P(*[q[3].data_ptr() for q in problems]),
        P(*[q[4].data_ptr() for q in problems]), L(*[q[4].stride(0) for q in problems]),
        L(*[q[0].shape[0] for q in problems]), L(*[q[2].shape[0] for q in problems]), K,
        F(*[float(q[5]) for q in problems]), I(*[int(bool(q[6])) for q in problems]), dy_fmt, x_fmt, int(split_accumulate),
        _stream(),
    )
    if gemm_timer is not None:
        e1.record()
        gemm_timer.append((sum(2.0 * K * q[0].shape[0] * q[2].shape[0] for q in problems), e0, e1))


def _req_slopes(alibi_slopes, n_heads: int) -> None:
    _req(alibi_slopes, torch.float32, "alibi_slopes")
    if alibi_slopes.numel() != n_heads or not alibi_slopes.is_contiguous():
        raise ValueError(f"alibi_slopes must be a contiguous fp32 [{n_heads}] tensor, got {tuple(alibi_slopes.shape)}")


def _attn_layout(qkv, n_heads: int, head_dim: int, **rows) -> None:
    if qkv.dim() != 2 or qkv.stride(1) != 1:
        raise ValueError(f"qkv must be a 2-D tensor with unit column stride, got strides {tuple(qkv.stride())}")
    T = qkv.shape[0]
    for name, t in rows.items():
        if tuple(t.shape) != (T, n_heads * head_dim) or not t.is_contiguous():
            raise ValueError(f"{name} must be a contiguous [{T}, {n_heads * head_dim}] tensor, got shape "
                             f"{tuple(t.shape)} strides {tuple(t.stride())}")


def _attn_lse_layout(lse, n_heads: int, T: int) -> None:
    if lse.dtype != torch.float32 or tuple(lse.shape) != (n_heads, T) or not lse.is_contiguous():
        raise ValueError(f"lse must be a contiguous fp32 [{n_heads}, {T}] tensor, got {lse.dtype} shape "
                         f"{tuple(lse.shape)} strides {tuple(lse.stride())}")


def _attn_dqkv(qkv, dqkv=None):
    if dqkv is None:
        return torch.empty_strided(qkv.shape, qkv.stride(), dtype=qkv.dtype, device=qkv.device)
    if dqkv.shape != qkv.shape or dqkv.stride() != qkv.stride():
        raise ValueError(f"dqkv must have qkv's shape {tuple(qkv.shape)} and strides {tuple(qkv.stride())}, got "
                         f"{tuple(dqkv.shape)} / {tuple(dqkv.stride())}")
    return dqkv


def attn_varlen_fwd(qkv, cu_seqlens, max_seqlen: int, n_groups: int, q_per_group: int, head_dim: int, scale: float, out=None,
                    dropout_p: float = 0.0, dropout_keys: tuple[int, int] = (0, 0), alibi_slopes=None):
    nh = n_groups * q_per_group
    _attn_layout(qkv, nh, head_dim, **({} if out is None else {"out": out}))
    _req(qkv, _BF16, "qkv"), _req(cu_seqlens, torch.int32, "cu_seqlens")
    if out is not None:
        _req(out, _BF16, "out")
    T = qkv.shape[0]
    o = torch.empty(T, nh * head_dim, dtype=_BF16, device=qkv.device) if out is None else out
    lse = torch.empty(nh, T, dtype=torch.float32, device=qkv.device)
    if alibi_slopes is not None:
        _req_slopes(alibi_slopes, nh)
        _lib.call(
            "dolomite_b200_attn_varlen_fwd_alibi", qkv.data_ptr(), qkv.stride(0), o.data_ptr(), lse.data_ptr(),
            cu_seqlens.data_ptr(), cu_seqlens.numel() - 1, T, int(max_seqlen), n_groups, q_per_group, head_dim, scale,
            float(dropout_p), dropout_keys[0], dropout_keys[1], alibi_slopes.data_ptr(), _stream(),
        )
        return o, lse
    if dropout_p:
        _lib.call(
            "dolomite_b200_attn_varlen_fwd_dropout", qkv.data_ptr(), qkv.stride(0), o.data_ptr(), lse.data_ptr(),
            cu_seqlens.data_ptr(), cu_seqlens.numel() - 1, T, int(max_seqlen), n_groups, q_per_group, head_dim, scale,
            float(dropout_p), dropout_keys[0], dropout_keys[1], _stream(),
        )
        return o, lse
    _lib.call(
        "dolomite_b200_attn_varlen_fwd", qkv.data_ptr(), qkv.stride(0), o.data_ptr(), lse.data_ptr(),
        cu_seqlens.data_ptr(), cu_seqlens.numel() - 1, T, int(max_seqlen), n_groups, q_per_group, head_dim, scale, _stream(),
    )
    return o, lse


def attn_varlen_bwd(dout, qkv, out, lse, cu_seqlens, max_seqlen, n_groups, q_per_group, head_dim, scale, dqkv=None,
                    dropout_p: float = 0.0, dropout_keys: tuple[int, int] = (0, 0), alibi_slopes=None):
    T = qkv.shape[0]
    _attn_layout(qkv, n_groups * q_per_group, head_dim, dout=dout, out=out)
    _attn_lse_layout(lse, n_groups * q_per_group, T)
    dqkv = _attn_dqkv(qkv, dqkv)
    _req(dout, _BF16, "dout"), _req(qkv, _BF16, "qkv"), _req(out, _BF16, "out"), _req(dqkv, _BF16, "dqkv")
    ws_bytes = _lib.load().dolomite_b200_attn_varlen_bwd_workspace_bytes(T, n_groups, q_per_group, head_dim)
    ws = _workspace(ws_bytes, qkv.device)
    if alibi_slopes is not None:
        _req_slopes(alibi_slopes, n_groups * q_per_group)
        _lib.call(
            "dolomite_b200_attn_varlen_bwd_alibi", dout.data_ptr(), qkv.data_ptr(), qkv.stride(0), out.data_ptr(),
            lse.data_ptr(), dqkv.data_ptr(), cu_seqlens.data_ptr(), cu_seqlens.numel() - 1, T, int(max_seqlen), n_groups,
            q_per_group, head_dim, scale, float(dropout_p), dropout_keys[0], dropout_keys[1], alibi_slopes.data_ptr(),
            ws.data_ptr(), _stream(),
        )
        return dqkv
    if dropout_p:
        _lib.call(
            "dolomite_b200_attn_varlen_bwd_dropout", dout.data_ptr(), qkv.data_ptr(), qkv.stride(0), out.data_ptr(),
            lse.data_ptr(), dqkv.data_ptr(), cu_seqlens.data_ptr(), cu_seqlens.numel() - 1, T, int(max_seqlen), n_groups,
            q_per_group, head_dim, scale, float(dropout_p), dropout_keys[0], dropout_keys[1], ws.data_ptr(), _stream(),
        )
        return dqkv
    _lib.call(
        "dolomite_b200_attn_varlen_bwd", dout.data_ptr(), qkv.data_ptr(), qkv.stride(0), out.data_ptr(), lse.data_ptr(),
        dqkv.data_ptr(), cu_seqlens.data_ptr(), cu_seqlens.numel() - 1, T, int(max_seqlen), n_groups, q_per_group,
        head_dim, scale, ws.data_ptr(), _stream(),
    )
    return dqkv


def attn_decode(qkv, k_cache, v_cache, lens, n_groups: int, q_per_group: int, head_dim: int, scale: float,
                alibi_slopes=None):
    _req(qkv, _BF16, "qkv"), _req(k_cache, _BF16, "k_cache"), _req(v_cache, _BF16, "v_cache"), _req(lens, torch.int32, "lens")
    B = qkv.shape[0]
    assert k_cache.shape == v_cache.shape and k_cache.shape[0] == B and k_cache.shape[2] == n_groups * head_dim
    assert k_cache.is_contiguous() and v_cache.is_contiguous() and qkv.stride(1) == 1
    out = torch.empty(B, n_groups * q_per_group * head_dim, dtype=_BF16, device=qkv.device)
    if alibi_slopes is not None:
        _req_slopes(alibi_slopes, n_groups * q_per_group)
        _lib.call("dolomite_b200_attn_decode_alibi", qkv.data_ptr(), qkv.stride(0), k_cache.data_ptr(), v_cache.data_ptr(),
                  lens.data_ptr(), out.data_ptr(), B, k_cache.shape[1], n_groups, q_per_group, head_dim, scale,
                  alibi_slopes.data_ptr(), _stream())
        return out
    _lib.call("dolomite_b200_attn_decode", qkv.data_ptr(), qkv.stride(0), k_cache.data_ptr(), v_cache.data_ptr(), lens.data_ptr(),
              out.data_ptr(), B, k_cache.shape[1], n_groups, q_per_group, head_dim, scale, _stream())
    return out


class MoEPlan:

    __slots__ = ("T", "E", "k", "max_rows", "sel_idx", "sel_w", "counts", "offsets", "tile_group", "cursors",
                 "row_of_slot", "slot_of_row", "token_of_row")


def moe_route(router_logits, k: int) -> MoEPlan:
    _req(router_logits, _BF16, "router_logits")
    T, E = router_logits.shape
    dev = router_logits.device
    p = MoEPlan()
    p.T, p.E, p.k = T, E, k
    p.max_rows = _lib.load().dolomite_b200_moe_max_rows(T, E, k)
    i32 = dict(dtype=torch.int32, device=dev)
    p.sel_idx = torch.empty(T, k, **i32)
    p.sel_w = torch.empty(T, k, dtype=torch.float32, device=dev)
    p.counts = torch.empty(E, **i32)
    p.offsets = torch.empty(E + 1, **i32)
    p.tile_group = torch.empty(p.max_rows // 128, **i32)
    p.cursors = torch.empty(E, **i32)
    p.row_of_slot = torch.empty(T * k, **i32)
    p.slot_of_row = torch.empty(p.max_rows, **i32)
    p.token_of_row = torch.empty(p.max_rows, **i32)
    _lib.call("dolomite_b200_moe_route", router_logits.data_ptr(), T, E, k, p.sel_idx.data_ptr(), p.sel_w.data_ptr(),
              p.counts.data_ptr(), p.offsets.data_ptr(), p.tile_group.data_ptr(), p.cursors.data_ptr(),
              p.row_of_slot.data_ptr(), p.slot_of_row.data_ptr(), p.token_of_row.data_ptr(), _stream())
    return p


def moe_gather(x, plan: MoEPlan):
    T, H = x.shape
    xg = torch.empty(plan.max_rows, H, dtype=_BF16, device=x.device)
    _lib.call("dolomite_b200_moe_gather", x.data_ptr(), xg.data_ptr(), plan.slot_of_row.data_ptr(), plan.offsets.data_ptr(),
              T, plan.E, plan.k, H, _stream())
    return xg


def moe_combine(yg, plan: MoEPlan, c=None, alpha: float = 1.0):
    H = yg.shape[1]
    out = torch.empty(plan.T, H, dtype=_BF16, device=yg.device)
    _lib.call("dolomite_b200_moe_combine", yg.data_ptr(), plan.row_of_slot.data_ptr(), plan.sel_w.data_ptr(), _ptr(c),
              out.data_ptr(), plan.T, plan.k, H, alpha, _stream())
    return out


def moe_combine_bwd(dy, yg, plan: MoEPlan, alpha: float = 1.0):
    H = yg.shape[1]
    dyg = torch.empty_like(yg)
    dw = torch.zeros(plan.T, plan.k, dtype=torch.float32, device=yg.device)
    _lib.call("dolomite_b200_moe_combine_bwd", dy.data_ptr(), yg.data_ptr(), plan.slot_of_row.data_ptr(),
              plan.offsets.data_ptr(), plan.sel_w.data_ptr(), dyg.data_ptr(), dw.data_ptr(), plan.T, plan.E, plan.k, H,
              alpha, _stream())
    return dyg, dw


def moe_token_sum(dxg, plan: MoEPlan):
    H = dxg.shape[1]
    dx = torch.empty(plan.T, H, dtype=_BF16, device=dxg.device)
    _lib.call("dolomite_b200_moe_token_sum", dxg.data_ptr(), plan.row_of_slot.data_ptr(), dx.data_ptr(), plan.T, plan.k, H, _stream())
    return dx


def moe_router_bwd(plan: MoEPlan, dw):
    dl = torch.empty(plan.T, plan.E, dtype=_BF16, device=dw.device)
    _lib.call("dolomite_b200_moe_router_bwd", plan.sel_idx.data_ptr(), plan.sel_w.data_ptr(), dw.data_ptr(), dl.data_ptr(),
              plan.T, plan.E, plan.k, _stream())
    return dl


def moe_aux_acc(E: int, device) -> torch.Tensor:
    return torch.zeros(2, E, dtype=torch.float32, device=device)


def moe_aux_stats(router_logits, plan: MoEPlan, T_real: int, acc) -> None:
    _req(router_logits, _BF16, "router_logits"), _req(acc, torch.float32, "acc")
    T, E = router_logits.shape
    assert router_logits.is_contiguous() and acc.is_contiguous() and acc.numel() == 2 * E and T == plan.T and E == plan.E
    n = _lib.load().dolomite_b200_moe_aux_partial_floats(T_real, E)
    partial = torch.empty(max(n, 1), dtype=torch.float32, device=acc.device)
    _lib.call("dolomite_b200_moe_aux_stats", router_logits.data_ptr(), plan.sel_idx.data_ptr(), T, T_real, E, plan.k,
              partial.data_ptr(), acc.data_ptr(), _stream())


def moe_aux_finalize(acc, n_tokens: int, coef: float = 0.0, loss=None):
    _req(acc, torch.float32, "acc")
    E = acc.shape[-1]
    if loss is not None:
        _req(loss, torch.float32, "loss")
        assert loss.numel() == 1
    aux = torch.empty(1, dtype=torch.float32, device=acc.device)
    c = torch.empty(E, dtype=torch.float32, device=acc.device)
    _lib.call("dolomite_b200_moe_aux_finalize", acc.data_ptr(), E, int(n_tokens), float(coef), aux.data_ptr(), c.data_ptr(),
              _ptr(loss), _stream())
    return aux, c


def moe_router_bwd_aux(router_logits, plan: MoEPlan, dw, c, s, T_real: int):
    _req(router_logits, _BF16, "router_logits"), _req(c, torch.float32, "c"), _req(s, torch.float32, "s")
    assert router_logits.is_contiguous() and tuple(router_logits.shape) == (plan.T, plan.E) and c.numel() == plan.E
    dl = torch.empty(plan.T, plan.E, dtype=_BF16, device=dw.device)
    _lib.call("dolomite_b200_moe_router_bwd_aux", router_logits.data_ptr(), plan.sel_idx.data_ptr(), plan.sel_w.data_ptr(),
              dw.data_ptr(), c.data_ptr(), s.data_ptr(), dl.data_ptr(), plan.T, T_real, plan.E, plan.k, _stream())
    return dl


def _expert_bias(bias, E: int, N: int):
    _req(bias, _BF16, "bias")
    assert bias.shape == (E, N) and bias.stride(1) == 1, (tuple(bias.shape), E, N)
    return bias


def gemm_grouped_m(a, w3, plan: MoEPlan, *, b_mn: bool, alpha: float = 1.0, flags=None, bias=None):
    _req(a, _BF16, "a"), _req(w3, _BF16, "w3")
    rows, K = a.shape
    E = w3.shape[0]
    N = w3.shape[2] if b_mn else w3.shape[1]
    assert (w3.shape[1] if b_mn else w3.shape[2]) == K and rows == plan.max_rows and w3.is_contiguous()
    out = torch.empty(rows, N, dtype=_BF16, device=a.device)
    if flags is None:
        flags = _default_gemm_flags
    if bias is not None:
        bias = _expert_bias(bias, E, N)
        _lib.call("dolomite_b200_gemm_bf16_grouped_m_bias", a.data_ptr(), a.stride(0), 0, None, w3.data_ptr(), w3.shape[2],
                  int(b_mn), out.data_ptr(), N, bias.data_ptr(), bias.stride(0), alpha, rows, N, K,
                  plan.tile_group.data_ptr(), E, flags, _stream())
        return out
    _lib.call("dolomite_b200_gemm_bf16_grouped_m", a.data_ptr(), a.stride(0), w3.data_ptr(), w3.shape[2], int(b_mn),
              out.data_ptr(), N, alpha, rows, N, K, plan.tile_group.data_ptr(), E, flags, _stream())
    return out


def gemm_grouped_m_gather(x, w3, plan: MoEPlan, alpha: float = 1.0, flags=None, bias=None):
    _req(x, _BF16, "x"), _req(w3, _BF16, "w3")
    T, K = x.shape
    E, N = w3.shape[0], w3.shape[1]
    assert w3.shape[2] == K and w3.is_contiguous() and x.stride(1) == 1 and T == plan.T
    out = torch.empty(plan.max_rows, N, dtype=_BF16, device=x.device)
    if flags is None:
        flags = _default_gemm_flags
    if gemm_timer is not None:
        e0, e1 = torch.cuda.Event(enable_timing=True), torch.cuda.Event(enable_timing=True)
        e0.record()
    if bias is not None:
        bias = _expert_bias(bias, E, N)
        _lib.call("dolomite_b200_gemm_bf16_grouped_m_bias", x.data_ptr(), x.stride(0), T, plan.token_of_row.data_ptr(),
                  w3.data_ptr(), w3.shape[2], 0, out.data_ptr(), N, bias.data_ptr(), bias.stride(0), alpha, plan.max_rows,
                  N, K, plan.tile_group.data_ptr(), E, flags, _stream())
    else:
        _lib.call("dolomite_b200_gemm_bf16_grouped_m_gather", x.data_ptr(), x.stride(0), T, plan.token_of_row.data_ptr(),
                  w3.data_ptr(), w3.shape[2], out.data_ptr(), N, alpha, plan.max_rows, N, K, plan.tile_group.data_ptr(), E,
                  flags, _stream())
    if gemm_timer is not None:
        e1.record()
        gemm_timer.append((2.0 * T * plan.k * N * K, e0, e1))
    return out


def gemm_grouped_k(a, b, plan: MoEPlan, out3, alpha: float = 1.0, beta: float = 1.0):
    _req(a, _BF16, "a"), _req(b, _BF16, "b"), _req(out3, torch.float32, "out3")
    rows, M = a.shape
    N = b.shape[1]
    assert out3.shape == (plan.E, M, N) and out3.is_contiguous()
    _lib.call("dolomite_b200_gemm_bf16_grouped_k", a.data_ptr(), a.stride(0), b.data_ptr(), b.stride(0), out3.data_ptr(), N,
              alpha, beta, M, N, rows, plan.offsets.data_ptr(), plan.E, _stream())
    return out3
```

include/dolomite_b200.h:

```cpp
#ifndef DOLOMITE_B200_H
#define DOLOMITE_B200_H

#include <stdint.h>

#ifdef __cplusplus
extern "C" {
#endif

#define DOLOMITE_B200_ABI_VERSION 1

#define DOLO_OK 0
#define DOLO_ERR_INVALID (-1)
#define DOLO_ERR_CUDA (-2)

const char* dolomite_b200_last_error(void);
int dolomite_b200_abi_version(void);
int dolomite_b200_device_info(int* sm_count, int* cc_major, int* cc_minor);
int dolomite_b200_set_option(const char* key, int value);
int dolomite_b200_get_option(const char* key, int* value);

int dolomite_b200_rmsnorm_fwd(const void* x, const void* w, void* y, float* rstd, int64_t T, int H, float eps,
                              void* stream);
int64_t dolomite_b200_rmsnorm_bwd_workspace_bytes(int H);
int dolomite_b200_rmsnorm_bwd(const void* dy, const void* x, const void* w, const float* rstd, const void* dx_add,
                              void* dx, float* dw_accum, void* workspace, int64_t T, int H, void* stream);

int dolomite_b200_rope_qk_inplace(void* qkv, int64_t row_stride, int64_t T, int n_groups, int q_per_group,
                                  int head_dim, const void* cos_table, const void* sin_table, const void* position_ids,
                                  int position_ids_is_int64, int64_t n_positions, int inverse, void* stream);

int dolomite_b200_layernorm_fwd(const void* x, const void* w, const void* b, void* y, float* mean, float* rstd, int64_t T,
                                int H, float eps, void* stream);
int64_t dolomite_b200_layernorm_bwd_workspace_bytes(int H);
int dolomite_b200_layernorm_bwd(const void* dy, const void* x, const void* w, const float* mean, const float* rstd,
                                const void* dx_add, void* dx, float* dw_accum, float* db_accum, void* workspace, int64_t T,
                                int H, void* stream);

enum {
    DOLO_ACT_CELU = 0,
    DOLO_ACT_ELU,
    DOLO_ACT_GELU,
    DOLO_ACT_GELU_TANH,
    DOLO_ACT_SELU,
    DOLO_ACT_HARDSHRINK,
    DOLO_ACT_HARDSIGMOID,
    DOLO_ACT_HARDSWISH,
    DOLO_ACT_HARDTANH,
    DOLO_ACT_LAPLACE,
    DOLO_ACT_LEAKY_RELU,
    DOLO_ACT_LOG_SIGMOID,
    DOLO_ACT_MISH,
    DOLO_ACT_RELU,
    DOLO_ACT_RELU2,
    DOLO_ACT_RELU6,
    DOLO_ACT_SIGMOID,
    DOLO_ACT_SILU,
    DOLO_ACT_SOFTPLUS,
    DOLO_ACT_SOFTSHRINK,
    DOLO_ACT_SOFTSIGN,
    DOLO_ACT_TANH,
    DOLO_ACT_TANHSHRINK,
    DOLO_ACT_COUNT
};
enum { DOLO_ACT_PLAIN = 0, DOLO_ACT_GLU = 1, DOLO_ACT_SIGMOID_GLU = 2 };
int dolomite_b200_act_fwd(int act_id, int form, const void* x, void* y, int64_t T, int64_t F, void* stream);
int dolomite_b200_act_bwd(int act_id, int form, const void* dy, const void* x, void* dx, float* dbias_accum, int64_t T,
                          int64_t F, void* stream);
int dolomite_b200_act_bwd_segmented(int act_id, int form, const void* dy, const void* x, void* dx, float* dbias_accum,
                                    int64_t ld_dbias, int64_t F, const int32_t* seg_offsets, int num_segments,
                                    void* stream);

int dolomite_b200_gelu_fwd(const void* x, void* y, int64_t n, void* stream);
int dolomite_b200_gelu_bwd(const void* dy, const void* x, void* dx, float* dbias_accum, int64_t T, int64_t F, void* stream);

int dolomite_b200_swiglu_fwd(const void* x, void* y, int64_t T, int64_t F, void* stream);
int dolomite_b200_swiglu_bwd(const void* dy, const void* x, void* dx, int64_t T, int64_t F, void* stream);
int dolomite_b200_swiglu_bwd_bias(const void* dy, const void* x, void* dx, float* dbias_accum, int64_t T, int64_t F,
                                  void* stream);

int dolomite_b200_embedding_fwd(const int64_t* ids, const void* wte, void* out, int64_t T, int H, int64_t V,
                                float scale, void* stream);
int dolomite_b200_embedding_bwd(const int64_t* ids, const void* dout, float* dwte, int64_t T, int H, int64_t V,
                                float scale, void* stream);

int dolomite_b200_cross_entropy_fwd_bwd(const void* logits, int64_t ldl, const int64_t* labels, void* dlogits,
                                        float* loss_per_token, float* loss_mean, float* scratch, int64_t T, int64_t V,
                                        int64_t ignore_index, float logit_scale, float grad_scale, void* stream);
int dolomite_b200_cross_entropy_count(const int64_t* labels, int64_t T, int64_t ignore_index, float* scratch,
                                      void* stream);
int dolomite_b200_cross_entropy_rows(const void* logits, int64_t ldl, const int64_t* labels, void* dlogits,
                                     float* loss_per_token, const float* scratch, int64_t T, int64_t V,
                                     int64_t ignore_index, float logit_scale, float grad_scale, void* stream);
int dolomite_b200_cross_entropy_mean(const float* loss_per_token, int64_t T, const float* scratch, float* loss_mean,
                                     void* stream);

int dolomite_b200_colsum_accum(const void* x, int64_t ldx, float* out, int64_t T, int64_t N, float scale,
                               void* stream);
int dolomite_b200_colsum_accum_segmented(const void* x, int64_t ldx, float* out, int64_t ld_out, int64_t N,
                                         const int32_t* seg_offsets, int num_segments, float scale, void* stream);
int dolomite_b200_scale_bf16_by_device_scalar(void* x, int64_t n, const float* scale, void* stream);

int dolomite_b200_add_scaled(const void* a, const void* b, void* out, float alpha, int64_t n, void* stream);

int dolomite_b200_dropout_fwd(const void* x, const void* residual, void* out, int64_t n, float p, float post_mul,
                              uint32_t key0, uint32_t key1, void* stream);
int dolomite_b200_dropout_bwd(const void* dy, void* dx, int64_t n, float p, float pre_mul, uint32_t key0, uint32_t key1,
                              void* stream);

int64_t dolomite_b200_sumsq_workspace_bytes(void);
int dolomite_b200_sumsq_accum(const float* g, int64_t n, float* out, void* workspace, void* stream);
int dolomite_b200_clip_coef(const float* sumsq, float max_norm, float* coef_out, float* norm_out, void* stream);
int dolomite_b200_adamw_step(float* p, const float* g, float* m, float* v, void* p_bf16, int64_t n, float lr,
                             float beta1, float beta2, float eps, float weight_decay, int64_t step,
                             const float* clip_coef, void* stream);
int dolomite_b200_cast_f32_to_bf16(const float* src, void* dst, int64_t n, void* stream);
int dolomite_b200_accum_bf16_into_f32(const void* src, float* dst, float scale, int64_t n, void* stream);

int dolomite_b200_attn_decode(const void* qkv, int64_t row_stride, const void* k_cache, const void* v_cache, const int32_t* lens,
                              void* out, int batch, int64_t L_max, int n_groups, int q_per_group, int head_dim,
                              float softmax_scale, void* stream);
int dolomite_b200_attn_decode_alibi(const void* qkv, int64_t row_stride, const void* k_cache, const void* v_cache,
                                    const int32_t* lens, void* out, int batch, int64_t L_max, int n_groups, int q_per_group,
                                    int head_dim, float softmax_scale, const float* alibi_slopes, void* stream);

#define DOLO_GEMM_FLAG_TMA_STORE 1
#define DOLO_GEMM_FLAG_SPLITK_ACCUMULATE 2
#define DOLO_GEMM_FLAG_CTA_PAIR 4
#define DOLO_GEMM_FLAG_NO_CTA_PAIR 8
#define DOLO_GEMM_FLAG_DIRECT_EPILOGUE 16
#define DOLO_GEMM_FLAG_F32_TMA_EPILOGUE 32
int dolomite_b200_gemm_bf16(const void* A, int64_t lda, int a_mn_major, const void* B, int64_t ldb, int b_mn_major,
                            void* D, int64_t ldd, int d_is_f32, const void* C, int64_t ldc, float alpha, float beta,
                            const void* bias, int64_t M, int64_t N, int64_t K, int flags, void* stream);

int dolomite_b200_gemm_bf16_wgrad_multi(int n_problems, const void* const* dY, const int64_t* ld_dy, const void* const* X,
                                        const int64_t* ld_x, float* const* dW, const int64_t* ld_dw, const int64_t* M,
                                        const int64_t* N, int64_t K, const float* alpha, const int* accumulate,
                                        void* stream);

int dolomite_b200_gemm_bf16_tile_n(int n_problems, const int64_t* M, const int64_t* N, int* tile_n,
                                   float* cost_256_over_128);

int dolomite_b200_gemm_fp8(const void* A, int64_t lda, int a_fmt, const void* B, int64_t ldb, int b_fmt,
                           const float* a_scale_inv, const float* b_scale_inv, void* D, int64_t ldd, int d_is_f32,
                           const void* C, int64_t ldc, float alpha, float beta, const void* bias, int64_t M, int64_t N,
                           int64_t K, int split_accumulate, void* stream);
int dolomite_b200_gemm_fp8_wgrad_multi(int n_problems, const void* const* dYt, const int64_t* ld_dyt, const void* const* Xt,
                                       const int64_t* ld_xt, const float* const* dy_scale_inv,
                                       const float* const* x_scale_inv, float* const* dW, const int64_t* ld_dw,
                                       const int64_t* M, const int64_t* N, int64_t K, const float* alpha,
                                       const int* accumulate, int dy_fmt, int x_fmt, int split_accumulate, void* stream);
int dolomite_b200_fp8_cast(const void* x, int64_t ldx, int64_t rows, int64_t cols, int fmt, const float* scale, void* out,
                           void* out_t, float* amax, void* stream);
int dolomite_b200_fp8_scaling_update(float* amax_history, int history_len, int64_t n_slots, float* scale, float* scale_inv,
                                     float fp8_max, void* stream);

int dolomite_b200_gemm_bf16_grouped_m(const void* A, int64_t lda, const void* B, int64_t ldb, int b_mn_major, void* D,
                                      int64_t ldd, float alpha, int64_t M_max, int64_t N, int64_t K,
                                      const int32_t* m_tile_group, int num_groups, int flags, void* stream);
int dolomite_b200_gemm_bf16_grouped_m_gather(const void* A, int64_t lda, int64_t a_rows, const int32_t* a_row_index,
                                             const void* B, int64_t ldb, void* D, int64_t ldd, float alpha, int64_t M_max,
                                             int64_t N, int64_t K, const int32_t* m_tile_group, int num_groups, int flags,
                                             void* stream);
int dolomite_b200_gemm_bf16_grouped_m_bias(const void* A, int64_t lda, int64_t a_rows, const int32_t* a_row_index,
                                           const void* B, int64_t ldb, int b_mn_major, void* D, int64_t ldd,
                                           const void* bias, int64_t ld_bias, float alpha, int64_t M_max, int64_t N,
                                           int64_t K, const int32_t* m_tile_group, int num_groups, int flags,
                                           void* stream);
int dolomite_b200_gemm_bf16_grouped_k(const void* A, int64_t lda, const void* B, int64_t ldb, float* D, int64_t ldd,
                                      float alpha, float beta, int64_t M, int64_t N, int64_t K_max,
                                      const int32_t* group_k_offsets, int num_groups, void* stream);

int64_t dolomite_b200_moe_max_rows(int64_t T, int E, int k);
int dolomite_b200_moe_route(const void* router_logits, int64_t T, int E, int k, int32_t* sel_idx, float* sel_w,
                            int32_t* counts, int32_t* offsets_padded, int32_t* m_tile_group, int32_t* cursors,
                            int32_t* row_of_slot, int32_t* slot_of_row, int32_t* token_of_row, void* stream);
int dolomite_b200_moe_gather(const void* x, void* xg, const int32_t* slot_of_row, const int32_t* offsets_padded,
                             int64_t T, int E, int k, int H, void* stream);
int dolomite_b200_moe_combine(const void* yg, const int32_t* row_of_slot, const float* sel_w, const void* c, void* out,
                              int64_t T, int k, int H, float alpha, void* stream);
int dolomite_b200_moe_combine_bwd(const void* dy, const void* yg, const int32_t* slot_of_row,
                                  const int32_t* offsets_padded, const float* sel_w, void* dyg, float* dw, int64_t T,
                                  int E, int k, int H, float alpha, void* stream);
int dolomite_b200_moe_token_sum(const void* dxg, const int32_t* row_of_slot, void* dx, int64_t T, int k, int H,
                                void* stream);
int dolomite_b200_moe_router_bwd(const int32_t* sel_idx, const float* sel_w, const float* dw, void* dlogits, int64_t T,
                                 int E, int k, void* stream);

int64_t dolomite_b200_moe_aux_partial_floats(int64_t T_real, int E);
int dolomite_b200_moe_aux_stats(const void* router_logits, const int32_t* sel_idx, int64_t T, int64_t T_real, int E, int k,
                                float* partial, float* acc, void* stream);
int dolomite_b200_moe_aux_finalize(const float* acc, int E, int64_t n_tokens, float coef, float* aux, float* c,
                                   float* loss, void* stream);
int dolomite_b200_moe_router_bwd_aux(const void* router_logits, const int32_t* sel_idx, const float* sel_w,
                                     const float* dw, const float* c, const float* s, void* dlogits, int64_t T,
                                     int64_t T_real, int E, int k, void* stream);

int dolomite_b200_attn_varlen_fwd(const void* qkv, int64_t row_stride, void* out, float* lse,
                                  const int32_t* cu_seqlens, int n_docs, int64_t T, int max_seqlen, int n_groups,
                                  int q_per_group, int head_dim, float softmax_scale, void* stream);
int64_t dolomite_b200_attn_varlen_bwd_workspace_bytes(int64_t T, int n_groups, int q_per_group, int head_dim);
int dolomite_b200_attn_varlen_bwd(const void* dout, const void* qkv, int64_t row_stride, const void* out,
                                  const float* lse, void* dqkv, const int32_t* cu_seqlens, int n_docs, int64_t T,
                                  int max_seqlen, int n_groups, int q_per_group, int head_dim, float softmax_scale,
                                  void* workspace, void* stream);
int dolomite_b200_attn_varlen_fwd_dropout(const void* qkv, int64_t row_stride, void* out, float* lse,
                                          const int32_t* cu_seqlens, int n_docs, int64_t T, int max_seqlen, int n_groups,
                                          int q_per_group, int head_dim, float softmax_scale, float dropout_p,
                                          uint32_t key0, uint32_t key1, void* stream);
int dolomite_b200_attn_varlen_bwd_dropout(const void* dout, const void* qkv, int64_t row_stride, const void* out,
                                          const float* lse, void* dqkv, const int32_t* cu_seqlens, int n_docs, int64_t T,
                                          int max_seqlen, int n_groups, int q_per_group, int head_dim,
                                          float softmax_scale, float dropout_p, uint32_t key0, uint32_t key1,
                                          void* workspace, void* stream);
int dolomite_b200_attn_varlen_fwd_alibi(const void* qkv, int64_t row_stride, void* out, float* lse,
                                        const int32_t* cu_seqlens, int n_docs, int64_t T, int max_seqlen, int n_groups,
                                        int q_per_group, int head_dim, float softmax_scale, float dropout_p, uint32_t key0,
                                        uint32_t key1, const float* alibi_slopes, void* stream);
int dolomite_b200_attn_varlen_bwd_alibi(const void* dout, const void* qkv, int64_t row_stride, const void* out,
                                        const float* lse, void* dqkv, const int32_t* cu_seqlens, int n_docs, int64_t T,
                                        int max_seqlen, int n_groups, int q_per_group, int head_dim, float softmax_scale,
                                        float dropout_p, uint32_t key0, uint32_t key1, const float* alibi_slopes,
                                        void* workspace, void* stream);

#ifdef __cplusplus
}
#endif
#endif
```

Measured before the change: 18330.

## Mix 256-wide and 128-wide tiles in one GEMM launch via makespan planner

Adds a planner that splits each problem's N dimension into a 256-wide tiled region and a 128-wide tail region, picking the split with a per-tile cost model and a wave makespan estimate. The persistent kernel enumerates wide tiles first and narrow tail tiles second, runs the narrow ones with a 128-wide accumulator and loads only half the B stage. This targets wave quantization and padding waste when the whole GEMM uses a single tile width. The cost is more complex tile indexing, two compiled mainloop/epilogue widths inside the 256 kernel, and reliance on a heuristic cost constant.

```diff
diff --git a/dolomite_engine_b200/_lib.py b/dolomite_engine_b200/_lib.py
--- a/dolomite_engine_b200/_lib.py
+++ b/dolomite_engine_b200/_lib.py
@@ -64,6 +64,7 @@
     ),
     "dolomite_b200_gemm_bf16_wgrad_multi": (_I, [_I, _P, _P, _P, _P, _P, _P, _P, _P, _L, _P, _P, _P]),
     "dolomite_b200_gemm_bf16_tile_n": (_I, [_I, _P, _P, _P, _P]),
+    "dolomite_b200_gemm_bf16_plan": (_I, [_I, _P, _P, _L, _I, _P, _P, _P]),
     "dolomite_b200_gemm_fp8": (
         _I,
         [_P, _L, _I, _P, _L, _I, _P, _P, _P, _L, _I, _P, _L, _F, _F, _P, _L, _L, _L, _I, _P],
@@ -160,6 +161,7 @@
     "dolomite_b200_attn_varlen_bwd": 3, "dolomite_b200_attn_varlen_fwd_dropout": 1, "dolomite_b200_attn_varlen_bwd_dropout": 3,
     "dolomite_b200_attn_varlen_fwd_alibi": 1, "dolomite_b200_attn_varlen_bwd_alibi": 3, "dolomite_b200_attn_decode_alibi": 1,
     "dolomite_b200_dropout_fwd": 1, "dolomite_b200_dropout_bwd": 1, "dolomite_b200_gemm_bf16_tile_n": 0,
+    "dolomite_b200_gemm_bf16_plan": 0,
     "dolomite_b200_moe_aux_stats": 2,
 }
 launch_counts: dict[str, int] = {}
diff --git a/dolomite_engine_b200/csrc/gemm.cu b/dolomite_engine_b200/csrc/gemm.cu
--- a/dolomite_engine_b200/csrc/gemm.cu
+++ b/dolomite_engine_b200/csrc/gemm.cu
@@ -38,6 +38,7 @@
 static_assert(PRODUCER_REGS * 128 + 2 * CONSUMER_REGS * 128 <= 65536, "register file exceeded");
 
 constexpr double TILE256_COST = 1.65;
+constexpr double NARROW_IN_WIDE_COST = 1.65;
 
 constexpr int MAXP = 4;
 
@@ -54,6 +55,7 @@
     int num_m, num_n, num_kb;
     int group_m;
     int tile_start;
+    int col1, num_n1, tile_start1;
     float alpha, beta;
     uint64_t hint_a, hint_b;
 };
@@ -62,6 +64,7 @@
     Problem pr[MAXP];
     int n_prob;
     int num_tiles;
+    int num_tiles0;
     int d_is_f32;
     int grouped;
     const int* m_tile_group;
@@ -79,7 +82,8 @@
 
 struct TileInfo {
     int q;
-    int m_blk, n_blk, grp, kb0, kb1;
+    int m_blk, col0, grp, kb0, kb1;
+    bool narrow;
     bool valid;
 };
 
@@ -93,23 +97,31 @@
     n_blk = r / gsize;
 }
 
-template <bool GROUPED>
+template <bool GROUPED, int TN>
 __device__ __forceinline__ TileInfo tile_info(int t, const GemmParams& p) {
     TileInfo ti;
+    ti.narrow = TN == 256 && t >= p.num_tiles0;
+    if (ti.narrow) t -= p.num_tiles0;
     ti.q = 0;
 #pragma unroll
     for (int i = 1; i < MAXP; ++i)
-        if (i < p.n_prob && t >= p.pr[i].tile_start) ti.q = i;
+        if (i < p.n_prob && t >= (ti.narrow ? p.pr[i].tile_start1 : p.pr[i].tile_start)) ti.q = i;
     const Problem& pr = p.pr[ti.q];
-    t -= pr.tile_start;
+    t -= ti.narrow ? pr.tile_start1 : pr.tile_start;
     ti.grp = 0;
     ti.kb0 = 0;
     ti.kb1 = pr.num_kb;
     ti.valid = true;
+    int n_blk;
+    if (TN == 256 && ti.narrow) {
+        tile_coords(t, pr.num_m, pr.num_n1, pr.group_m, ti.m_blk, n_blk);
+        ti.col0 = pr.col1 + n_blk * 128;
+        return ti;
+    }
     if (GROUPED && p.grouped == 3) {
         const int per = pr.num_m * pr.num_n;
         const int split = t / per;
-        tile_coords(t - split * per, pr.num_m, pr.num_n, pr.group_m, ti.m_blk, ti.n_blk);
+        tile_coords(t - split * per, pr.num_m, pr.num_n, pr.group_m, ti.m_blk, n_blk);
         const int kb_per = (pr.num_kb + p.num_groups - 1) / p.num_groups;
         ti.kb0 = split * kb_per;
         ti.kb1 = min(pr.num_kb, ti.kb0 + kb_per);
@@ -117,17 +129,18 @@
     } else if (GROUPED && p.grouped == 2) {
         const int per = pr.num_m * pr.num_n;
         ti.grp = t / per;
-        tile_coords(t - ti.grp * per, pr.num_m, pr.num_n, pr.group_m, ti.m_blk, ti.n_blk);
+        tile_coords(t - ti.grp * per, pr.num_m, pr.num_n, pr.group_m, ti.m_blk, n_blk);
         ti.kb0 = p.group_k_offsets[ti.grp] / BK;
         ti.kb1 = p.group_k_offsets[ti.grp + 1] / BK;
         ti.valid = ti.kb1 > ti.kb0;
     } else {
-        tile_coords(t, pr.num_m, pr.num_n, pr.group_m, ti.m_blk, ti.n_blk);
+        tile_coords(t, pr.num_m, pr.num_n, pr.group_m, ti.m_blk, n_blk);
         if (GROUPED && p.grouped == 1) {
             ti.grp = p.m_tile_group[ti.m_blk];
             ti.valid = ti.grp >= 0;
         }
     }
+    ti.col0 = n_blk * TN;
     return ti;
 }
 
@@ -291,12 +304,16 @@
     }
 };
 
+template <int W>
+struct TileWidth {
+    static constexpr int value = W;
+};
+
 template <class Op, int TN>
 __device__ __forceinline__ void gemm_body(const GemmMaps& maps, const GemmParams& p) {
     constexpr bool A_MN = Op::A_MN, B_MN = Op::B_MN;
     constexpr int STAGES = Ring<TN>::STAGES;
     constexpr int B_STAGE_BYTES = Ring<TN>::B_BYTES;
-    constexpr int STAGE_BYTES = Ring<TN>::STAGE_BYTES;
     extern __shared__ uint8_t smem_raw[];
     uint8_t* smem = smem_align_1024(smem_raw);
     uint8_t* smem_a = smem;
@@ -334,7 +351,7 @@
             int stage = 0;
             uint32_t phase = 0;
             for (int t = blockIdx.x; t < num_tiles; t += gridDim.x) {
-                const TileInfo ti = tile_info<Op::GROUPED>(t, p);
+                const TileInfo ti = tile_info<Op::GROUPED, TN>(t, p);
                 if (!ti.valid) continue;
                 const CUtensorMap* tmap_b = &maps.b[ti.q];
                 const int b_outer = ti.grp * p.b_group_rows;
@@ -347,11 +364,11 @@
                     if (lane == 0) {
                         mbar_expect_tx(&full_bar[stage], B_STAGE_BYTES);
                         if (!B_MN) {
-                            tma_load_2d(sb, tmap_b, &full_bar[stage], kb * BK, b_outer + ti.n_blk * BN);
+                            tma_load_2d(sb, tmap_b, &full_bar[stage], kb * BK, b_outer + ti.col0);
                         } else {
 #pragma unroll
                             for (int i = 0; i < BN / 64; ++i)
-                                tma_load_2d(sb + i * (BK * 128), tmap_b, &full_bar[stage], ti.n_blk * BN + i * 64,
+                                tma_load_2d(sb + i * (BK * 128), tmap_b, &full_bar[stage], ti.col0 + i * 64,
                                             b_outer + kb * BK);
                         }
                     }
@@ -375,18 +392,19 @@
             int stage = 0;
             uint32_t phase = 0;
             for (int t = blockIdx.x; t < num_tiles; t += gridDim.x) {
-                const TileInfo ti = tile_info<Op::GROUPED>(t, p);
+                const TileInfo ti = tile_info<Op::GROUPED, TN>(t, p);
                 if (!ti.valid) continue;
                 const CUtensorMap* tmap_a = &maps.a[ti.q];
                 const CUtensorMap* tmap_b = &maps.b[ti.q];
                 const uint64_t ha = p.pr[ti.q].hint_a, hb = p.pr[ti.q].hint_b;
-                const int m_blk = ti.m_blk, n_blk = ti.n_blk;
+                const int m_blk = ti.m_blk, col0 = ti.col0;
                 const int b_outer = (Op::GROUPED && p.grouped == 1) ? ti.grp * p.b_group_rows : 0;
+                const int width = TN == 256 && ti.narrow ? 128 : TN;
                 for (int kb = ti.kb0; kb < ti.kb1; ++kb) {
                     mbar_wait(&empty_bar[stage], phase ^ 1, 1);
                     uint8_t* sa = smem_a + stage * A_STAGE_BYTES;
                     uint8_t* sb = smem_b + stage * B_STAGE_BYTES;
-                    mbar_expect_tx(&full_bar[stage], STAGE_BYTES);
+                    mbar_expect_tx(&full_bar[stage], A_STAGE_BYTES + width * BK * 2);
                     if (!A_MN) {
                         tma_load_2d_hint(sa, tmap_a, &full_bar[stage], kb * Op::KB_ELEMS, m_blk * BM, ha);
                     } else {
@@ -395,12 +413,17 @@
                             tma_load_2d_hint(sa + i * (BK * 128), tmap_a, &full_bar[stage], m_blk * BM + i * 64, kb * BK, ha);
                     }
                     if (!B_MN) {
-                        tma_load_2d_hint(sb, tmap_b, &full_bar[stage], kb * Op::KB_ELEMS, b_outer + n_blk * TN, hb);
+#pragma unroll
+                        for (int i = 0; i < TN / 128; ++i)
+                            if (i * 128 < width)
+                                tma_load_2d_hint(sb + i * (128 * 128), tmap_b, &full_bar[stage], kb * Op::KB_ELEMS,
+                                                 b_outer + col0 + i * 128, hb);
                     } else {
 #pragma unroll
                         for (int i = 0; i < TN / 64; ++i)
-                            tma_load_2d_hint(sb + i * (BK * 128), tmap_b, &full_bar[stage], n_blk * TN + i * 64,
-                                             b_outer + kb * BK, hb);
+                            if (i * 64 < width)
+                                tma_load_2d_hint(sb + i * (BK * 128), tmap_b, &full_bar[stage], col0 + i * 64,
+                                                 b_outer + kb * BK, hb);
                     }
                     if (++stage == STAGES) { stage = 0; phase ^= 1; }
                 }
@@ -424,10 +447,10 @@
     float acc[TN / 2];
     float tot[TN / 2];
     for (int t = blockIdx.x; t < num_tiles; t += gridDim.x) {
-        const TileInfo ti = tile_info<Op::GROUPED>(t, p);
+        const TileInfo ti = tile_info<Op::GROUPED, TN>(t, p);
         const Problem& pr = p.pr[ti.q];
         const int row0 = ti.m_blk * BM + cw * 64;
-        const int col0 = ti.n_blk * TN;
+        const int col0 = ti.col0;
         const int dgrp = Op::GROUPED && p.grouped == 2 ? ti.grp : 0;
         if (!ti.valid) {
             if (Op::GROUPED && p.grouped == 2 && p.d_is_f32 && pr.C == nullptr) epi.store_zero_f32<TN>(&maps.d[ti.q], col0, row0, dgrp);
@@ -435,65 +458,78 @@
         }
         const bool has_bias = pr.bias != nullptr;
         const bool has_c = pr.C != nullptr;
-        uint32_t bias_v = 0;
-        if (has_bias && wt < TN / 2 && col0 + 2 * wt < pr.N) {
-            const __nv_bfloat16* brow = pr.bias + ti.grp * p.bias_group_stride;
-            if (col0 + 2 * wt + 1 < pr.N)
-                bias_v = __ldg(reinterpret_cast<const uint32_t*>(brow + col0 + 2 * wt));
+        auto tile = [&](auto width) {
+            constexpr int W = decltype(width)::value;
+            float(&a)[W / 2] = reinterpret_cast<float(&)[W / 2]>(acc);
+            float(&tw)[W / 2] = reinterpret_cast<float(&)[W / 2]>(tot);
+            uint32_t bias_v = 0;
+            if (has_bias && wt < W / 2 && col0 + 2 * wt < pr.N) {
+                const __nv_bfloat16* brow = pr.bias + ti.grp * p.bias_group_stride;
+                if (col0 + 2 * wt + 1 < pr.N)
+                    bias_v = __ldg(reinterpret_cast<const uint32_t*>(brow + col0 + 2 * wt));
+                else
+                    bias_v = __bfloat16_as_ushort(brow[col0 + 2 * wt]);
+            }
+            [[maybe_unused]] int prev_stage = -1;
+            for (int kb = ti.kb0; kb < ti.kb1; ++kb) {
+                mbar_wait(&full_bar[stage], phase, 3);
+                wgmma_fence();
+                const uint32_t sa = smem_u32(smem_a + stage * A_STAGE_BYTES);
+                const uint32_t sb = smem_u32(smem_b + stage * B_STAGE_BYTES);
+#pragma unroll
+                for (int k = 0; k < 4; ++k) {
+                    const uint64_t adesc = A_MN ? gmma_desc(sa + cw * (BK * 128) + k * 2048, BK * 128, 1024, 1)
+                                                : gmma_desc(sa + cw * (64 * 128) + k * 32, 16, 1024, 1);
+                    const uint64_t bdesc = B_MN ? gmma_desc(sb + k * 2048, BK * 128, 1024, 1)
+                                                : gmma_desc(sb + k * 32, 16, 1024, 1);
+                    Op::template mma<W>(a, adesc, bdesc, ((!Op::SPLIT && kb != ti.kb0) || k != 0) ? 1u : 0u);
+                }
+                wgmma_commit();
+                if (kb == min(ti.kb0 + 2, ti.kb1 - 1) && has_c && epi.leader) epi.load_c_prefetch(&maps.c[ti.q], chunk_cols, col0, row0, dgrp);
+                if constexpr (Op::SPLIT) {
+                    wgmma_wait<0>();
+                    reg_fence<W / 2>(a);
+                    if (lane == 0) mbar_arrive(&empty_bar[stage]);
+                    if (kb == ti.kb0) {
+#pragma unroll
+                        for (int i = 0; i < W / 2; ++i) tw[i] = a[i];
+                    } else {
+#pragma unroll
+                        for (int i = 0; i < W / 2; ++i) tw[i] += a[i];
+                    }
+                } else {
+                    wgmma_wait<1>();
+                    if (prev_stage >= 0 && lane == 0) mbar_arrive(&empty_bar[prev_stage]);
+                    prev_stage = stage;
+                }
+                if (++stage == STAGES) { stage = 0; phase ^= 1; }
+            }
+            if constexpr (!Op::SPLIT) {
+                wgmma_wait<0>();
+                reg_fence<W / 2>(a);
+                if (prev_stage >= 0 && lane == 0) mbar_arrive(&empty_bar[prev_stage]);
+            }
+            const float(&res)[W / 2] = Op::SPLIT ? tw : a;
+            float s = 1.f;
+            if constexpr (Op::SCALED) s = __ldg(p.a_scale_inv[ti.q]) * __ldg(p.b_scale_inv[ti.q]);
+            if (has_bias && wt < W / 2) epi.bias[wt] = bias_v;
+            epi.begin_tile();
+
+            if (p.d_is_f32)
+                epi.store<W, true, Op::SCALED>(res, &maps.d[ti.q], &maps.c[ti.q], col0, row0, dgrp, s, pr.alpha, pr.beta,
+                                               has_bias, has_c, Op::GROUPED && p.grouped == 3);
             else
-                bias_v = __bfloat16_as_ushort(brow[col0 + 2 * wt]);
-        }
-        int prev_stage = -1;
-        for (int kb = ti.kb0; kb < ti.kb1; ++kb) {
-            mbar_wait(&full_bar[stage], phase, 3);
-            wgmma_fence();
-            const uint32_t sa = smem_u32(smem_a + stage * A_STAGE_BYTES);
-            const uint32_t sb = smem_u32(smem_b + stage * B_STAGE_BYTES);
-#pragma unroll
-            for (int k = 0; k < 4; ++k) {
-                const uint64_t adesc = A_MN ? gmma_desc(sa + cw * (BK * 128) + k * 2048, BK * 128, 1024, 1)
-                                            : gmma_desc(sa + cw * (64 * 128) + k * 32, 16, 1024, 1);
-                const uint64_t bdesc = B_MN ? gmma_desc(sb + k * 2048, BK * 128, 1024, 1)
-                                            : gmma_desc(sb + k * 32, 16, 1024, 1);
-                Op::template mma<TN>(acc, adesc, bdesc, ((!Op::SPLIT && kb != ti.kb0) || k != 0) ? 1u : 0u);
-            }
-            wgmma_commit();
-            if (kb == min(ti.kb0 + 2, ti.kb1 - 1) && has_c && epi.leader) epi.load_c_prefetch(&maps.c[ti.q], chunk_cols, col0, row0, dgrp);
-            if constexpr (Op::SPLIT) {
-                wgmma_wait<0>();
-                reg_fence<TN / 2>(acc);
-                if (lane == 0) mbar_arrive(&empty_bar[stage]);
-                if (kb == ti.kb0) {
-#pragma unroll
-                    for (int i = 0; i < TN / 2; ++i) tot[i] = acc[i];
-                } else {
-#pragma unroll
-                    for (int i = 0; i < TN / 2; ++i) tot[i] += acc[i];
-                }
-            } else {
-                wgmma_wait<1>();
-                if (prev_stage >= 0 && lane == 0) mbar_arrive(&empty_bar[prev_stage]);
-                prev_stage = stage;
-            }
-            if (++stage == STAGES) { stage = 0; phase ^= 1; }
-        }
-        if constexpr (!Op::SPLIT) {
-            wgmma_wait<0>();
-            reg_fence<TN / 2>(acc);
-            if (prev_stage >= 0 && lane == 0) mbar_arrive(&empty_bar[prev_stage]);
-        }
-        const float(&res)[TN / 2] = Op::SPLIT ? tot : acc;
-        float s = 1.f;
-        if constexpr (Op::SCALED) s = __ldg(p.a_scale_inv[ti.q]) * __ldg(p.b_scale_inv[ti.q]);
-        if (has_bias && wt < TN / 2) epi.bias[wt] = bias_v;
-        epi.begin_tile();
-
-        if (p.d_is_f32)
-            epi.store<TN, true, Op::SCALED>(res, &maps.d[ti.q], &maps.c[ti.q], col0, row0, dgrp, s, pr.alpha, pr.beta,
-                                            has_bias, has_c, Op::GROUPED && p.grouped == 3);
-        else
-            epi.store<TN, false, Op::SCALED>(res, &maps.d[ti.q], &maps.c[ti.q], col0, row0, dgrp, s, pr.alpha, pr.beta,
-                                             has_bias, has_c, false);
+                epi.store<W, false, Op::SCALED>(res, &maps.d[ti.q], &maps.c[ti.q], col0, row0, dgrp, s, pr.alpha, pr.beta,
+                                                has_bias, has_c, false);
+        };
+        if constexpr (TN == 256) {
+            if (ti.narrow)
+                tile(TileWidth<128>());
+            else
+                tile(TileWidth<256>());
+        } else {
+            tile(TileWidth<TN>());
+        }
     }
     if (epi.leader) tma_store_wait_all<0>();
 }
@@ -530,10 +566,7 @@
     return DOLO_OK;
 }
 
-int choose_tile_n(int n, const int64_t* M, const int64_t* N) {
-    const int forced = dolo_option_gemm_tile_n();
-    if (forced != 0) return forced;
-    const int64_t w = gemm_workers();
+int choose_tile_n(int n, const int64_t* M, const int64_t* N, int64_t w) {
     int64_t t128 = 0, t256 = 0;
     for (int q = 0; q < n; ++q) {
         const int64_t mb = (M[q] + BM - 1) / BM;
@@ -543,6 +576,84 @@
     const double c128 = double((t128 + w - 1) / w);
     const double c256 = double((t256 + w - 1) / w) * TILE256_COST;
     return c256 < c128 ? 256 : 128;
+}
+
+double makespan(int nseg, const int64_t* count, const double* cost, int64_t w) {
+    double base = 0.0;
+    int64_t first[2 * MAXP], extra[2 * MAXP], start = 0;
+    for (int i = 0; i < nseg; ++i) {
+        base += double(count[i] / w) * cost[i];
+        first[i] = start % w;
+        extra[i] = count[i] % w;
+        start += count[i];
+    }
+    double most = 0.0;
+    for (int i = 0; i < nseg; ++i) {
+        if (extra[i] == 0) continue;
+        double e = 0.0;
+        for (int j = 0; j < nseg; ++j)
+            if (extra[j] > 0 && (first[i] >= first[j] ? first[i] - first[j] : first[i] - first[j] + w) < extra[j]) e += cost[j];
+        most = e > most ? e : most;
+    }
+    return base + most;
+}
+
+struct GemmPlan {
+    int tile_n;
+    int64_t wide_cols[MAXP];
+    double cost, cost128, cost256;
+};
+
+GemmPlan plan_launch(int n, const int64_t* M, const int64_t* N, int64_t K, int64_t w, int forced) {
+    GemmPlan pl;
+    pl.tile_n = forced != 0 ? forced : choose_tile_n(n, M, N, w);
+    const double kb = double((K + BK - 1) / BK);
+    int64_t mb[MAXP], nb[MAXP], cnt[2 * MAXP];
+    double cost[2 * MAXP];
+    for (int q = 0; q < n; ++q) {
+        mb[q] = (M[q] + BM - 1) / BM;
+        nb[q] = (N[q] + 255) / 256;
+        pl.wide_cols[q] = N[q];
+        cnt[q] = mb[q] * ((N[q] + 127) / 128);
+        cost[q] = kb / TILE256_COST;
+    }
+    pl.cost128 = makespan(n, cnt, cost, w);
+    for (int q = 0; q < n; ++q) {
+        cnt[q] = mb[q] * nb[q];
+        cost[q] = kb;
+    }
+    pl.cost256 = makespan(n, cnt, cost, w);
+    pl.cost = pl.tile_n == 256 ? pl.cost256 : pl.cost128;
+    if (pl.tile_n != 256 || forced != 0) return pl;
+    int jmax[MAXP], j[MAXP] = {0, 0, 0, 0};
+    for (int q = 0; q < n; ++q) {
+        int64_t lim = (w + mb[q] - 1) / mb[q];
+        if (n > 1 && lim > 3) lim = 3;
+        jmax[q] = int(nb[q] < lim ? nb[q] : lim);
+    }
+    int64_t best_narrow = 0;
+    for (;;) {
+        int q = 0;
+        while (q < n && j[q] == jmax[q]) j[q++] = 0;
+        if (q == n) break;
+        ++j[q];
+        int64_t narrow = 0;
+        for (int i = 0; i < n; ++i) {
+            const int64_t wide = j[i] == 0 ? N[i] : (nb[i] - j[i]) * 256;
+            cnt[i] = mb[i] * ((wide + 255) / 256);
+            cost[i] = kb;
+            cnt[n + i] = mb[i] * ((N[i] - (wide < N[i] ? wide : N[i]) + 127) / 128);
+            cost[n + i] = kb / NARROW_IN_WIDE_COST;
+            narrow += cnt[n + i];
+        }
+        const double c = makespan(2 * n, cnt, cost, w);
+        if (c < pl.cost - 1e-9 || (c < pl.cost + 1e-9 && narrow < best_narrow)) {
+            pl.cost = c;
+            best_narrow = narrow;
+            for (int i = 0; i < n; ++i) pl.wide_cols[i] = j[i] == 0 ? N[i] : (nb[i] - j[i]) * 256;
+        }
+    }
+    return pl;
 }
 
 }
@@ -573,7 +684,7 @@
 };
 
 static int setup_problem(GemmMaps& maps, GemmParams& p, int q, const GemmProblemArgs& g, int ab, int a_mn_major,
-                         int b_mn_major, int d_is_f32, const GroupArgs& ga, int tile_n) {
+                         int b_mn_major, int d_is_f32, const GroupArgs& ga, int tile_n, int64_t wide_cols) {
     const int64_t M = g.M, N = g.N, K = g.K;
     if (ab == 1) {
         DOLO_REQUIRE(M > 0 && N > 0 && K > 0, "gemm_fp8: empty problem (M=%lld N=%lld K=%lld)", (long long)M,
@@ -622,7 +733,7 @@
     strides[0] = ab;
     if (!b_mn_major) {
         dims[0] = uint64_t(K); dims[1] = uint64_t(ga.mode == 1 ? ga.b_total_outer : N); strides[1] = uint64_t(g.ldb) * ab;
-        box[0] = 128 / ab; box[1] = uint32_t(tile_n);
+        box[0] = 128 / ab; box[1] = BN;
     } else {
         dims[0] = uint64_t(N); dims[1] = uint64_t(ga.mode == 1 ? ga.b_total_outer : K); strides[1] = uint64_t(g.ldb) * 2;
         box[0] = 64; box[1] = BK;
@@ -662,7 +773,13 @@
         pr.hint_b = a_smaller ? TMA_HINT_EVICT_FIRST : TMA_HINT_EVICT_LAST;
     }
     pr.num_m = int((M + BM - 1) / BM);
-    pr.num_n = int((N + tile_n - 1) / tile_n);
+    DOLO_REQUIRE(tile_n == 256 || wide_cols >= N, "gemm: 128-wide tiles only follow the wide tiles of a 128 x 256 launch");
+    if (wide_cols > N) wide_cols = N;
+    DOLO_REQUIRE(wide_cols == N || (wide_cols >= 0 && wide_cols % 256 == 0), "gemm: wide_cols=%lld must be a multiple of 256",
+                 (long long)wide_cols);
+    pr.num_n = int((wide_cols + tile_n - 1) / tile_n);
+    pr.col1 = int(wide_cols);
+    pr.num_n1 = int((N - wide_cols + 127) / 128);
     pr.num_kb = int((K * ab + 127) / 128);
     {
         const int64_t panel_bytes = int64_t(BM) * K * ab;
@@ -674,6 +791,20 @@
     return DOLO_OK;
 }
 
+static void enumerate_tiles(GemmParams& p, int n_prob, int groups) {
+    int t0 = 0, t1 = 0;
+    for (int q = 0; q < n_prob; ++q) {
+        Problem& pr = p.pr[q];
+        pr.tile_start = t0;
+        pr.tile_start1 = t1;
+        t0 += pr.num_m * pr.num_n * groups;
+        t1 += pr.num_m * pr.num_n1;
+    }
+    p.n_prob = n_prob;
+    p.num_tiles0 = t0;
+    p.num_tiles = t0 + t1;
+}
+
 template <int TN>
 static int dispatch_layout(int a_mn_major, int b_mn_major, const GemmMaps& maps, const GemmParams& p, cudaStream_t st) {
     if (!a_mn_major && !b_mn_major) return launch_gemm<TN, gemm_bf16_kernel<false, false, TN>>(maps, p, st);
@@ -707,16 +838,20 @@
     if (M == 0 || N == 0) return DOLO_OK;
     const bool tma_store = (flags & DOLO_GEMM_FLAG_TMA_STORE) != 0;
     DOLO_REQUIRE(!tma_store || (!d_is_f32 && C == nullptr), "gemm: TMA-store epilogue needs bf16 D and no C");
-    const int tile_n = ga.mode == 0 ? choose_tile_n(1, &M, &N) : BN;
+    int tile_n = BN;
+    int64_t wide_cols = N;
+    if (ga.mode == 0) {
+        const GemmPlan pl = plan_launch(1, &M, &N, K, gemm_workers(), dolo_option_gemm_tile_n());
+        tile_n = pl.tile_n;
+        wide_cols = pl.wide_cols[0];
+    }
     GemmMaps maps;
     GemmParams p;
     memset(&p, 0, sizeof(p));
     GemmProblemArgs g{A, lda, B, ldb, D, ldd, C, ldc, bias, alpha, beta, M, N, K};
-    int rc = setup_problem(maps, p, 0, g, 2, a_mn_major, b_mn_major, d_is_f32, ga, tile_n);
+    int rc = setup_problem(maps, p, 0, g, 2, a_mn_major, b_mn_major, d_is_f32, ga, tile_n, wide_cols);
     if (rc) return rc;
-    p.n_prob = 1;
-    p.pr[0].tile_start = 0;
-    p.num_tiles = p.pr[0].num_m * p.pr[0].num_n * (ga.mode >= 2 ? ga.num_groups : 1);
+    enumerate_tiles(p, 1, ga.mode >= 2 ? ga.num_groups : 1);
     p.d_is_f32 = d_is_f32;
     p.grouped = ga.mode;
     p.m_tile_group = ga.m_tile_group;
@@ -734,33 +869,46 @@
                                                    const float* alpha, const int* accumulate, void* stream) {
     DOLO_REQUIRE(n_problems >= 1 && n_problems <= MAXP, "wgrad_multi: between 1 and %d problems per launch", MAXP);
     for (int q = 0; q < n_problems; ++q) DOLO_REQUIRE(M[q] > 0 && N[q] > 0, "wgrad_multi: empty problem %d", q);
-    const int tile_n = choose_tile_n(n_problems, M, N);
+    const GemmPlan pl = plan_launch(n_problems, M, N, K, gemm_workers(), dolo_option_gemm_tile_n());
     GemmMaps maps;
     GemmParams p;
     memset(&p, 0, sizeof(p));
-    int tiles = 0;
     for (int q = 0; q < n_problems; ++q) {
         GemmProblemArgs g{dY[q], ld_dy[q], X[q], ld_x[q], dW[q], ld_dw[q], accumulate[q] ? dW[q] : nullptr, ld_dw[q], nullptr,
                           alpha[q], 1.f, M[q], N[q], K};
-        int rc = setup_problem(maps, p, q, g, 2, 1, 1, 1, GroupArgs(), tile_n);
+        int rc = setup_problem(maps, p, q, g, 2, 1, 1, 1, GroupArgs(), pl.tile_n, pl.wide_cols[q]);
         if (rc) return rc;
-        p.pr[q].tile_start = tiles;
-        tiles += p.pr[q].num_m * p.pr[q].num_n;
-    }
-    p.n_prob = n_problems;
-    p.num_tiles = tiles;
+    }
+    enumerate_tiles(p, n_problems, 1);
     p.d_is_f32 = 1;
     p.grouped = 0;
     p.num_groups = 1;
-    return dispatch(tile_n, 1, 1, maps, p, static_cast<cudaStream_t>(stream));
+    return dispatch(pl.tile_n, 1, 1, maps, p, static_cast<cudaStream_t>(stream));
 }
 
 extern "C" int dolomite_b200_gemm_bf16_tile_n(int n_problems, const int64_t* M, const int64_t* N, int* tile_n,
                                               float* cost_256_over_128) {
     DOLO_REQUIRE(n_problems >= 1 && n_problems <= MAXP && M != nullptr && N != nullptr && tile_n != nullptr,
                  "gemm_bf16_tile_n: between 1 and %d problems, non-null M, N and tile_n", MAXP);
-    *tile_n = choose_tile_n(n_problems, M, N);
+    const int forced = dolo_option_gemm_tile_n();
+    *tile_n = forced != 0 ? forced : choose_tile_n(n_problems, M, N, gemm_workers());
     if (cost_256_over_128 != nullptr) *cost_256_over_128 = float(TILE256_COST);
+    return DOLO_OK;
+}
+
+extern "C" int dolomite_b200_gemm_bf16_plan(int n_problems, const int64_t* M, const int64_t* N, int64_t K, int workers,
+                                            int* tile_n, int64_t* wide_cols, double* cost) {
+    DOLO_REQUIRE(n_problems >= 1 && n_problems <= MAXP && M != nullptr && N != nullptr && tile_n != nullptr &&
+                     wide_cols != nullptr && cost != nullptr,
+                 "gemm_bf16_plan: between 1 and %d problems, non-null M, N, tile_n, wide_cols and cost", MAXP);
+    DOLO_REQUIRE(K > 0 && workers >= 0, "gemm_bf16_plan: K > 0 and workers >= 0 needed");
+    for (int q = 0; q < n_problems; ++q) DOLO_REQUIRE(M[q] > 0 && N[q] > 0, "gemm_bf16_plan: empty problem %d", q);
+    const GemmPlan pl = plan_launch(n_problems, M, N, K, workers > 0 ? workers : gemm_workers(), dolo_option_gemm_tile_n());
+    *tile_n = pl.tile_n;
+    for (int q = 0; q < n_problems; ++q) wide_cols[q] = pl.wide_cols[q] < N[q] ? pl.wide_cols[q] : N[q];
+    cost[0] = pl.cost;
+    cost[1] = pl.cost128;
+    cost[2] = pl.cost256;
     return DOLO_OK;
 }
 
@@ -872,10 +1020,9 @@
     GemmParams p;
     memset(&p, 0, sizeof(p));
     GemmProblemArgs g{A, lda, B, ldb, D, ldd, C, ldc, bias, alpha, beta, M, N, K, a_scale_inv, b_scale_inv};
-    int rc = setup_problem(maps, p, 0, g, 1, 0, 0, d_is_f32, GroupArgs(), BN);
+    int rc = setup_problem(maps, p, 0, g, 1, 0, 0, d_is_f32, GroupArgs(), BN, N);
     if (rc) return rc;
-    p.n_prob = 1;
-    p.num_tiles = p.pr[0].num_m * p.pr[0].num_n;
+    enumerate_tiles(p, 1, 1);
     p.d_is_f32 = d_is_f32;
     p.num_groups = 1;
     return dispatch_fp8(a_fmt, b_fmt, split_accumulate, maps, p, static_cast<cudaStream_t>(stream));
@@ -893,17 +1040,13 @@
     GemmMaps maps;
     GemmParams p;
     memset(&p, 0, sizeof(p));
-    int tiles = 0;
     for (int q = 0; q < n_problems; ++q) {
         GemmProblemArgs g{dYt[q], ld_dyt[q], Xt[q], ld_xt[q], dW[q], ld_dw[q], accumulate[q] ? dW[q] : nullptr, ld_dw[q],
                           nullptr, alpha[q], 1.f, M[q], N[q], K, dy_scale_inv[q], x_scale_inv[q]};
-        int rc = setup_problem(maps, p, q, g, 1, 0, 0, 1, GroupArgs(), BN);
+        int rc = setup_problem(maps, p, q, g, 1, 0, 0, 1, GroupArgs(), BN, N[q]);
         if (rc) return rc;
-        p.pr[q].tile_start = tiles;
-        tiles += p.pr[q].num_m * p.pr[q].num_n;
-    }
-    p.n_prob = n_problems;
-    p.num_tiles = tiles;
+    }
+    enumerate_tiles(p, n_problems, 1);
     p.d_is_f32 = 1;
     p.num_groups = 1;
     return dispatch_fp8(dy_fmt, x_fmt, split_accumulate, maps, p, static_cast<cudaStream_t>(stream));
diff --git a/dolomite_engine_b200/kernels.py b/dolomite_engine_b200/kernels.py
--- a/dolomite_engine_b200/kernels.py
+++ b/dolomite_engine_b200/kernels.py
@@ -421,6 +421,17 @@
     return int(tile_n.value), float(cost.value)
 
 
+def gemm_plan(shapes: list[tuple[int, int]], K: int, workers: int = 0) -> dict:
+    import ctypes
+
+    n = len(shapes)
+    tile_n, wide, cost = ctypes.c_int(0), (ctypes.c_int64 * n)(), (ctypes.c_double * 3)()
+    _lib.call("dolomite_b200_gemm_bf16_plan", n, (ctypes.c_int64 * n)(*[s[0] for s in shapes]),
+              (ctypes.c_int64 * n)(*[s[1] for s in shapes]), int(K), int(workers), ctypes.addressof(tile_n),
+              ctypes.addressof(wide), ctypes.addressof(cost))
+    return {"tile_n": int(tile_n.value), "wide_cols": list(wide), "cost": cost[0], "cost_128": cost[1], "cost_256": cost[2]}
+
+
 E4M3, E5M2 = 0, 1
 FP8_MAX = {E4M3: 448.0, E5M2: 57344.0}
 _U8 = torch.uint8
diff --git a/include/dolomite_b200.h b/include/dolomite_b200.h
--- a/include/dolomite_b200.h
+++ b/include/dolomite_b200.h
@@ -141,6 +141,9 @@
 int dolomite_b200_gemm_bf16_tile_n(int n_problems, const int64_t* M, const int64_t* N, int* tile_n,
                                    float* cost_256_over_128);
 
+int dolomite_b200_gemm_bf16_plan(int n_problems, const int64_t* M, const int64_t* N, int64_t K, int workers,
+                                 int* tile_n, int64_t* wide_cols, double* cost);
+
 int dolomite_b200_gemm_fp8(const void* A, int64_t lda, int a_fmt, const void* B, int64_t ldb, int b_fmt,
                            const float* a_scale_inv, const float* b_scale_inv, void* D, int64_t ldd, int d_is_f32,
                            const void* C, int64_t ldc, float alpha, float beta, const void* bias, int64_t M, int64_t N,
```

New measurement: 18560 (median of 6 runs). 1.01x the previous value.
